# mit-han-lab/TinyChatEngine

Hardware: AMD Instinct MI355X
Metric: decode tokens/s (W4A16 linears of one token, M=1) + GEMV GB/s vs HBM roofline (higher is better)
Workload: dtype int4 weights x fp16 activations, fp32 accumulate; 1 GPU; W4A16 decode GEMV M=1, llama3-8b (true shapes, model.h:83): 32 blocks x [qkv [4096, 1024, 1024], o 4096, gate/up 14336, down] + lm_head 128256, group 128; parallelism=single GPU, issue=one hipGraph replay per token (129 launches in stream order)

## Files before the change

### tinychatengine_amd/csrc/tce_capi.hip

```cpp
#include <hip/hip_runtime.h>

#include <cstdarg>
#include <cstdio>
#include <cstring>
#include <new>
#include <algorithm>
#include <string>
#include <vector>

#include "tce_common.hpp"
#include "w4a16_kernels.hpp"

namespace tce {
int launch_w8a8(const tce_w8a8_desc &d, hipStream_t stream, hipError_t *hip_err, void *scratch = nullptr, char *describe = nullptr, int describe_len = 0);
size_t w8a8_scratch_bytes();
void set_w8a8_xsplit(int xs);
}

namespace {

thread_local char g_err[512] = "";
thread_local int g_gemv_rows = 0, g_gemv_wn = 0, g_gemv_wk = 0, g_gemv_depth = 0;
thread_local int g_gemm_mt = 0, g_gemm_nt = 0;
thread_local int g_debug_mode_capi = 0;
void *g_dbg_buf_capi = nullptr;

int fail(int code, const char *fmt, ...) __attribute__((format(printf, 2, 3)));
int fail(int code, const char *fmt, ...) {
    va_list ap;
    va_start(ap, fmt);
    vsnprintf(g_err, sizeof(g_err), fmt, ap);
    va_end(ap);
    return code;
}

int hip_fail(hipError_t e, const char *what) {
    return fail(TCE_ERR_HIP, "%s: %s", what, hipGetErrorString(e));
}

int check_w4a16(const tce_w4a16_desc *d) {
    if (!d) return fail(TCE_ERR_BAD_ARG, "null descriptor");
    if (!d->A || !d->qweight || !d->scales || !d->zeros || !d->C) return fail(TCE_ERR_BAD_ARG, "null data pointer");
    if (d->M <= 0 || d->N <= 0 || d->K <= 0) return fail(TCE_ERR_BAD_ARG, "non-positive M/N/K (%d,%d,%d)", d->M, d->N, d->K);
    if (d->group_size != 128 && d->group_size != 64 && d->group_size != 32)
        return fail(TCE_ERR_UNSUPPORTED_GROUP, "Unsupported group size: %d", d->group_size);
    if (d->K % d->group_size != 0 || d->K % 32 != 0)
        return fail(TCE_ERR_UNSUPPORTED_SHAPE, "K=%d must be a multiple of the group size and of 32", d->K);
    const int lda = d->lda ? d->lda : d->K;
    if (lda % 8 != 0 || reinterpret_cast<uintptr_t>(d->A) % 16 != 0)
        return fail(TCE_ERR_UNSUPPORTED_SHAPE, "A must be 16-byte aligned with lda %% 8 == 0");
    if (reinterpret_cast<uintptr_t>(d->qweight) % 16 != 0) return fail(TCE_ERR_UNSUPPORTED_SHAPE, "qweight must be 16-byte aligned");
    if (d->flags & TCE_W4_SILU_MUL_PAIRS) {
        if (d->N % 2 != 0) return fail(TCE_ERR_UNSUPPORTED_SHAPE, "TCE_W4_SILU_MUL_PAIRS needs an even N (interleaved gate/up rows), got %d", d->N);
        if (d->flags & (TCE_W4_ADD_TO_C | TCE_W4_FORCE_GEMM)) return fail(TCE_ERR_BAD_ARG, "TCE_W4_SILU_MUL_PAIRS cannot be combined with ADD_TO_C / FORCE_GEMM");
    }
    if (d->rmsnorm_gamma && (d->flags & TCE_W4_FORCE_GEMM)) return fail(TCE_ERR_BAD_ARG, "rmsnorm_gamma cannot be combined with TCE_W4_FORCE_GEMM");
    return TCE_OK;
}

}

extern "C" {

int tce_version(void) { return TCE_VERSION; }
const char *tce_last_error(void) { return g_err; }
const char *tce_build_info(void) { return "tce_hip gfx950 wave64 hipcc " __VERSION__; }

int64_t tce_w4a16_algorithmic_bytes(int M, int N, int K, int G) {
    const int64_t nk = (int64_t)N * K;
    return nk / 2 + 2 * nk / G + nk / (2 * (int64_t)G) + 2 * (int64_t)M * K + 2 * (int64_t)M * N;
}

thread_local int g_pk_mode = 0;
constexpr int kPkMinM = 129;

static bool use_pk(const tce_w4a16_desc *d, bool want_gemm) {
    if (!d->prepacked || g_pk_mode == 9 || !want_gemm || d->K % 128 != 0 || d->rmsnorm_gamma) return false;
    if (g_pk_mode >= 1 && g_pk_mode <= 8) return true;
    if (d->M < kPkMinM || g_gemm_mt != 0) return false;
    if (d->flags & TCE_W4_SILU_MUL_PAIRS) return true;
    if (d->group_size != 128) return true;
    const bool has_scratch = d->scratch != nullptr && (reinterpret_cast<uintptr_t>(d->scratch) & 255) == 0;
    return tce::gemm_pk_estimate_us(d->M, d->N, d->K, nullptr, has_scratch, nullptr, d->group_size, (d->flags & TCE_W4_ZERO_POINT_IS_8) != 0) < tce::gemm_dma_estimate_us(d->M, d->N, d->K) + 1.5f;
}

constexpr long long kPersistentMinWeights = 1LL << 62;
constexpr long long kFusedNormPersistentRows = 16384;
thread_local int g_gemv_kernel = 0;
thread_local int g_skinny_enabled = 1;

int tce_w4a16_set_gemv_config(int rows, int wn, int wk, int depth) {
    if (rows == 0 && wn == 0 && wk == 0) {
        g_gemv_rows = g_gemv_wn = g_gemv_wk = g_gemv_depth = 0;
        g_gemv_kernel = 0;
        tce::set_gemv_stream_config(0, 0, 0);
        return TCE_OK;
    }
    if (wk == 0) {
        if ((rows % 10 != 0 && rows % 10 != 1 && rows % 10 != 2 && rows % 10 != 4) || rows < 0 || rows >= 90 || wn < 1 || wn > 16 || (depth != 0 && depth != 2 && depth != 3))
            return fail(TCE_ERR_BAD_ARG, "stream GEMV config rows=%d waves=%d depth=%d is not available", rows, wn, depth);
        tce::set_gemv_stream_config(rows, wn, depth);
        g_gemv_kernel = 2;
        return TCE_OK;
    }
    const int dd = depth ? depth : 2;
    if (!tce::gemv_variant_exists(rows, wn, wk, dd))
        return fail(TCE_ERR_BAD_ARG, "GEMV variant rows=%d wn=%d wk=%d depth=%d was not compiled", rows, wn, wk, dd);
    g_gemv_rows = rows;
    g_gemv_wn = wn;
    g_gemv_wk = wk;
    g_gemv_depth = dd;
    g_gemv_kernel = 1;
    return TCE_OK;
}

int tce_w4a16_set_gemv_i8(int mode, int rows) {
    if (mode < 0 || mode > 1 || rows < 0 || rows > 2) return fail(TCE_ERR_BAD_ARG, "tce_w4a16_set_gemv_i8: mode %d rows %d", mode, rows);
    tce::set_gemv_i8_mode(mode, rows);
    return TCE_OK;
}

int tce_attention_set_tuning(int waves_per_workgroup, int workgroups, int heads_per_workgroup) {
    const bool ok = (waves_per_workgroup == 0 || waves_per_workgroup == 4 || waves_per_workgroup == 8 || waves_per_workgroup == 16) &&
                    (workgroups == 0 || (workgroups >= 32 && workgroups <= 8192)) &&
                    (heads_per_workgroup == 0 || heads_per_workgroup == 1 || heads_per_workgroup == 2 || heads_per_workgroup == 4);
    if (!ok) return fail(TCE_ERR_BAD_ARG, "tce_attention_set_tuning(%d, %d, %d)", waves_per_workgroup, workgroups, heads_per_workgroup);
    tce::set_attention_fast_waves(waves_per_workgroup);
    tce::set_attention_fast_target(workgroups);
    tce::set_attention_fast_fuse(heads_per_workgroup);
    return TCE_OK;
}

int tce_w8a8_set_tuning(int quartets_per_tile, int big_tiles, int deep_pipeline) {
    const bool ok = (quartets_per_tile == 0 || quartets_per_tile == 1 || quartets_per_tile == 2 || quartets_per_tile == 4) &&
                    ((big_tiles >= 0 && big_tiles <= 4) || big_tiles == 9) &&
                    (deep_pipeline == 0 || deep_pipeline == 1 || deep_pipeline == 2 || deep_pipeline == 4 || deep_pipeline == 9);
    if (!ok) return fail(TCE_ERR_BAD_ARG, "tce_w8a8_set_tuning(%d, %d, %d)", quartets_per_tile, big_tiles, deep_pipeline);
    tce::set_w8a8_ksplit(quartets_per_tile);
    tce::set_w8a8_big(big_tiles);
    tce::set_w8a8_deep(deep_pipeline);
    return TCE_OK;
}

static thread_local int g_plan_eager = 0;
int tce_w4a16_set_debug_mode(int mode) {
    if (mode >= 50000 && mode <= 50499) {
        tce::set_gemv_ovl_config((mode - 50000) % 100, (mode - 50000) / 100);
        return TCE_OK;
    }
    if (mode == 2930 || mode == 2931) {
        tce::set_attention_fast_probe_no_combine(mode - 2930);
        return TCE_OK;
    }
    if (mode >= 2920 && mode <= 2924) {
        tce::set_attention_fast_fuse(mode - 2920);
        return TCE_OK;
    }
    if (mode >= 2900 && mode <= 2916) {
        tce::set_attention_fast_waves(mode - 2900);
        return TCE_OK;
    }
    const bool pk_mode_in_attention_range = (mode >= 6950 && mode <= 6958) || (mode >= 6972 && mode <= 6974) || (mode >= 7700 && mode <= 7710 + 512) || mode == 6916 || mode == 6917;
    if (mode >= 3000 && mode <= 3000 + 8192 && !pk_mode_in_attention_range) {
        tce::set_attention_fast_target(mode - 3000);
        return TCE_OK;
    }
    if (mode >= 1000 && mode <= 1256) {
        tce::set_skinny_max_m(mode - 1000);
        return TCE_OK;
    }
    if (mode >= 2700 && mode <= 2899 && ((mode - 2700) % 100 == 0 || (mode - 2700) % 100 == 4 || (mode - 2700) % 100 == 8)) {
        tce::set_attention_prefill_waves((mode >= 2800 ? 200 : 100) + (mode % 100));
        return TCE_OK;
    }
    if (mode == 2950 || mode == 2954 || mode == 2958 || mode == 2964 || mode == 2968) {
        tce::set_attention_prefill_waves(mode - 2950);
        return TCE_OK;
    }
    if ((mode >= 75 && mode <= 78) || mode == 176 || mode == 177) {
        tce::set_w8a8_big(mode == 78 ? 9 : (mode >= 176 ? mode - 173 : mode - 75));
        return TCE_OK;
    }
    if (mode >= 7710 && mode <= 7710 + 512) {
        tce::set_i8_token_max_units(mode - 7710);
        return TCE_OK;
    }
    if (mode >= 7700 && mode <= 7703) {
        if (mode <= 7701) tce::set_i8_token_mode(mode - 7700);
        else {
#ifndef TCE_LAB
            if (mode == 7702) return fail(TCE_ERR_BAD_ARG, "debug mode 7702 (per-stage stamps of the token kernel) needs the lab build (python -m tinychatengine_amd.build --lab, TCE_LIB_PATH)");
#endif
            tce::set_i8_token_stamps(mode == 7702 ? g_dbg_buf_capi : nullptr);
        }
        return TCE_OK;
    }
    if (mode >= 19000 && mode <= 19999) {
        tce::set_w8a8_kslice(mode - 19000);
        return TCE_OK;
    }
    if (mode >= 190 && mode <= 192) {
        tce::set_w8a8_rows32(mode - 190);
        return TCE_OK;
    }
    if (mode >= 180 && mode <= 188) {
        tce::set_w8a8_xsplit(mode - 180);
        return TCE_OK;
    }
    if (mode == 170 || mode == 171 || mode == 172 || mode == 174 || mode == 179) {
        tce::set_w8a8_deep(mode - 170);
        return TCE_OK;
    }
    if (mode == 15000 || mode == 15001) {
        g_plan_eager = mode - 15000;
        return TCE_OK;
    }
    if (mode >= 70 && mode <= 74) {
        tce::set_w8a8_ksplit(mode - 70);
        return TCE_OK;
    }
    if (mode >= 640 && mode <= 644) {
        g_pk_mode = 4;
        tce::set_gemm_pk_ablation(0);
        tce::set_gemm_pk_mode(4, 0);
        tce::set_gemm_pk_split(mode - 640);
        return TCE_OK;
    }
#ifndef TCE_LAB
    if ((mode > 2600 && mode <= 2664) || (mode > 600 && mode <= 664) || (mode > 26000 && mode <= 26256) || mode == 1 || mode == 2 || mode == 4 || mode == 7702)
        return fail(TCE_ERR_BAD_ARG, "debug mode %d selects a diagnostic instantiation that only the lab build holds (python -m tinychatengine_amd.build --lab, TCE_LIB_PATH)", mode);
#endif
    if (mode >= 2600 && mode <= 2664) {
        g_pk_mode = mode == 2600 ? 0 : 6;
        tce::set_gemm_pk_mode(mode == 2600 ? 0 : 6, 0);
        tce::set_gemm_pk_ablation(mode - 2600);
        return TCE_OK;
    }
    if (mode >= 600 && mode <= 664) {
        g_pk_mode = mode == 600 ? 0 : 1;
        tce::set_gemm_pk_mode(mode == 600 ? 0 : 1, 0);
        tce::set_gemm_pk_ablation(mode - 600);
        return TCE_OK;
    }
    if (mode == 2676) {
        g_pk_mode = 8;
        tce::set_gemm_pk_ablation(0);
        tce::set_gemm_pk_split(0);
        tce::set_gemm_pk_mode(16, 0);
        return TCE_OK;
    }
    if (mode >= 51000 && mode <= 51016) {
        tce::set_gemv_i8_mixed_waves(mode - 51000);
        return TCE_OK;
    }
    if (mode == 6916 || mode == 6917) {
        tce::set_gemm_pk_form16_auto(mode - 6916);
        return TCE_OK;
    }
    if (mode == 2675) {
        g_pk_mode = 8;
        tce::set_gemm_pk_ablation(0);
        tce::set_gemm_pk_split(0);
        tce::set_gemm_pk_mode(15, 0);
        return TCE_OK;
    }
    if (mode == 2673 || mode == 2674) {
        g_pk_mode = 8;
        tce::set_gemm_pk_ablation(0);
        tce::set_gemm_pk_split(0);
        tce::set_gemm_pk_mode(mode - 2660, 0);
        return TCE_OK;
    }
    if (mode >= 2670 && mode <= 2672) {
        g_pk_mode = 8;
        tce::set_gemm_pk_ablation(0);
        tce::set_gemm_pk_split(0);
        tce::set_gemm_pk_mode(10 + mode - 2670, 0);
        return TCE_OK;
    }
    if (mode >= 2682 && mode <= 2684) {
        g_pk_mode = 8;
        tce::set_gemm_pk_ablation(0);
        tce::set_gemm_pk_mode(12, 0);
        tce::set_gemm_pk_split(mode - 2680);
        return TCE_OK;
    }
    if (mode >= 6950 && mode <= 6958) {
        tce::set_gemm_pk_handoff_delta(mode - 6950);
        return TCE_OK;
    }
    if (mode == 696 || mode == 697 || mode == 698 || (mode >= 6972 && mode <= 6974)) {
        tce::set_gemm_pk_prio(mode == 698 ? -1 : mode >= 6970 ? mode - 6970 : mode - 696);
        return TCE_OK;
    }
    if (mode == 694 || mode == 695) {
        tce::set_gemm_pk_handoff(mode - 694);
        return TCE_OK;
    }
    if (mode == 692 || mode == 693) {
        tce::set_gemm_pk_wide_auto(mode - 692);
        return TCE_OK;
    }
    if (mode >= 26000 && mode <= 26256) {
        g_pk_mode = mode == 26000 ? 0 : 8;
        tce::set_gemm_pk_mode(mode == 26000 ? 0 : 10, 0);
        tce::set_gemm_pk_ablation(mode - 26000);
        return TCE_OK;
    }
    if (mode == 2669) {
        g_pk_mode = 8;
        tce::set_gemm_pk_ablation(0);
        tce::set_gemm_pk_split(0);
        tce::set_gemm_pk_mode(9, 0);
        return TCE_OK;
    }
    if (mode >= 672 && mode <= 674) {
        g_pk_mode = 7;
        tce::set_gemm_pk_ablation(0);
        tce::set_gemm_pk_mode(7, 0);
        tce::set_gemm_pk_split(mode - 670);
        return TCE_OK;
    }
    if (mode == 690 || mode == 691) {
        tce::set_gemm_pk256_auto(mode - 690);
        return TCE_OK;
    }
    if (mode >= 60 && mode <= 69) {
        g_pk_mode = mode - 60;
        tce::set_gemm_pk_split(0);
        tce::set_gemm_pk_ablation(0);
        tce::set_gemm_pk_mode(g_pk_mode >= 1 && g_pk_mode <= 8 && g_pk_mode != 5 ? g_pk_mode : 0, 0);
        return TCE_OK;
    }
    if (mode >= 50 && mode <= 52) {
        tce::set_gemm_dma_mode(mode - 50);
        return TCE_OK;
    }
    if (mode == 40 || mode == 41 || mode == 42 || mode == 44 || mode == 48) {
        tce::set_gemm_xcd_rows(mode - 40);
        tce::set_gemm_dma_xcd_rows(mode - 40);
        return TCE_OK;
    }
    if (mode >= 45 && mode <= 47) {
        tce::set_gemv_shared_xsum(mode == 45 ? 2 : mode - 46);
        return TCE_OK;
    }
    if (mode >= 80 && mode <= 87) {
        tce::set_lnq_form(mode - 80);
        return TCE_OK;
    }
    if (mode >= 20 && mode <= 30) {
        g_skinny_enabled = mode != 29;
        tce::set_skinny_config(mode == 29 ? 0 : (mode == 30 ? 9 : mode - 20));
        return TCE_OK;
    }
    if (mode >= 10 && mode <= 12) {
        tce::set_gemv_order(mode - 10);
        return TCE_OK;
    }
    if (mode < 0 || mode > 4) return fail(TCE_ERR_BAD_ARG, "debug mode %d", mode);
    tce::set_gemv_debug_mode(mode);
    tce::set_gemv_stream_debug(mode, g_dbg_buf_capi);
    tce::set_gemv_ovl_stamps(mode == 2 ? g_dbg_buf_capi : nullptr);
    g_debug_mode_capi = mode;
    return TCE_OK;
}

int tce_w4a16_set_debug_buffer(void *buf) {
    tce::set_lnq_stamps(buf);
    tce::set_gemv_debug_buffer(buf);
    g_dbg_buf_capi = buf;
    tce::set_gemv_stream_debug(g_debug_mode_capi, buf);
    tce::set_gemv_ovl_stamps(g_debug_mode_capi == 2 ? buf : nullptr);
    return TCE_OK;
}

int tce_reset_last_error(void) {
    int first = 0;
    for (int i = 0; i < 8; ++i) {
        const hipError_t e = hipGetLastError();
        if (e == hipSuccess) break;
        if (!first) first = (int)e;
    }
    fail(TCE_OK, "");
    return first;
}

int tce_malloc(void **ptr, size_t bytes, int managed) {
    if (!ptr || bytes == 0) return fail(TCE_ERR_BAD_ARG, "tce_malloc: bad argument");
    const hipError_t e = managed ? hipMallocManaged(ptr, bytes, hipMemAttachGlobal) : hipMalloc(ptr, bytes);
    return e == hipSuccess ? TCE_OK : hip_fail(e, managed ? "hipMallocManaged" : "hipMalloc");
}

int tce_free(void *ptr) {
    if (!ptr) return TCE_OK;
    const hipError_t e = hipFree(ptr);
    return e == hipSuccess ? TCE_OK : hip_fail(e, "hipFree");
}

int tce_host_alloc(void **ptr, size_t bytes) {
    if (!ptr || bytes == 0) return fail(TCE_ERR_BAD_ARG, "tce_host_alloc: bad argument");
    const hipError_t e = hipHostMalloc(ptr, bytes, hipHostMallocMapped | hipHostMallocCoherent);
    return e == hipSuccess ? TCE_OK : hip_fail(e, "hipHostMalloc");
}

int tce_host_free(void *ptr) {
    if (!ptr) return TCE_OK;
    const hipError_t e = hipHostFree(ptr);
    return e == hipSuccess ? TCE_OK : hip_fail(e, "hipHostFree");
}

int tce_memcpy(void *dst, const void *src, size_t bytes, int kind, void *stream) {
    if (!dst || !src) return fail(TCE_ERR_BAD_ARG, "tce_memcpy: null pointer");
    const hipMemcpyKind k = kind == TCE_MEMCPY_H2D ? hipMemcpyHostToDevice : (kind == TCE_MEMCPY_D2H ? hipMemcpyDeviceToHost : hipMemcpyDeviceToDevice);
    const hipError_t e = hipMemcpyAsync(dst, src, bytes, k, static_cast<hipStream_t>(stream));
    return e == hipSuccess ? TCE_OK : hip_fail(e, "hipMemcpyAsync");
}

int tce_synchronize(void *stream) {
    const hipError_t e = stream ? hipStreamSynchronize(static_cast<hipStream_t>(stream)) : hipDeviceSynchronize();
    return e == hipSuccess ? TCE_OK : hip_fail(e, "synchronize");
}

int tce_device_count(void) {
    int n = 0;
    return hipGetDeviceCount(&n) == hipSuccess ? n : 0;
}

int tce_w4a16_gemv_variant(int idx, int *rows, int *wn, int *wk, int *depth) {
    static const int table[][4] = {
#define TCE_V(R, N_, K_, D_) {R, N_, K_, D_},
        TCE_GEMV_VARIANTS(TCE_V)
#undef TCE_V
    };
    const int n = (int)(sizeof(table) / sizeof(table[0]));
    if (idx < 0 || idx >= n || !rows || !wn || !wk || !depth) return TCE_ERR_BAD_ARG;
    *rows = table[idx][0];
    *wn = table[idx][1];
    *wk = table[idx][2];
    *depth = table[idx][3];
    return TCE_OK;
}

int tce_w4a16_gemm_variant(int idx, int *mt, int *nt) {
    static const int table[][2] = {
#define TCE_V(M_, N_) {M_, N_}, {100 + M_, N_}, {200 + M_, N_},
        TCE_GEMM_VARIANTS(TCE_V)
#undef TCE_V
    };
    const int n = (int)(sizeof(table) / sizeof(table[0]));
    if (idx < 0 || idx >= n || !mt || !nt) return TCE_ERR_BAD_ARG;
    *mt = table[idx][0];
    *nt = table[idx][1];
    return TCE_OK;
}

int tce_w4a16_set_gemm_config(int mt, int nt) {
    if (mt == 0 && nt == 0) {
        g_gemm_mt = g_gemm_nt = 0;
        return TCE_OK;
    }
    if (!tce::gemm_variant_exists(mt >= 200 ? mt - 200 : mt, nt)) return fail(TCE_ERR_BAD_ARG, "GEMM variant %dx%d was not compiled", mt, nt);
    g_gemm_mt = mt;
    g_gemm_nt = nt;
    return TCE_OK;
}

static int forward_group_norm(const tce_w4a16_desc *descs, int count, const float *gamma, float eps, void *stream) {
    if (!descs || count < 1 || count > TCE_MAX_GROUP) return fail(TCE_ERR_BAD_ARG, "group count %d not in 1..%d", count, TCE_MAX_GROUP);
    if (!gamma || reinterpret_cast<uintptr_t>(gamma) % 16 != 0) return fail(TCE_ERR_BAD_ARG, "gamma must be a 16-byte aligned fp32 [K] vector");
    for (int i = 0; i < count; ++i) {
        const int rc = check_w4a16(&descs[i]);
        if (rc != TCE_OK) return rc;
        const tce_w4a16_desc &a = descs[0], &b = descs[i];
        if (b.M != a.M || b.K != a.K || b.group_size != a.group_size || b.A != a.A || b.lda != a.lda)
            return fail(TCE_ERR_BAD_ARG, "grouped linears must share M, K, group size and the activation");
    }
    if (descs[0].M != 1) return fail(TCE_ERR_UNSUPPORTED_SHAPE, "the fused RMSNorm prologue is a decode (M = 1) path; use tce_rmsnorm_half for M = %d", descs[0].M);
    hipError_t he = hipSuccess;
    if (g_gemv_kernel == 0 && g_debug_mode_capi == 0 && tce::gemv_i8_supports(descs, count, true)) {
        const int rc = tce::launch_w4a16_gemv_i8(descs, count, static_cast<hipStream_t>(stream), &he, gamma, eps);
        if (rc == TCE_OK) return TCE_OK;
        if (rc == TCE_ERR_HIP) return hip_fail(he, "w4a16 gemv (int8 contraction, rmsnorm prologue) launch");
        if (rc != TCE_ERR_UNSUPPORTED_SHAPE) return fail(rc, "w4a16 gemv (int8 contraction, rmsnorm prologue): unsupported configuration");
    }
    long long rows = 0;
    for (int i = 0; i < count; ++i) rows += descs[i].N;
// ... 897 lines not shown
    return rc == TCE_OK ? TCE_OK : fail(rc, "%s: unsupported shape", who);
}

int tce_layernorm_q_w8a8_group(const float *x, const float *ln_weight, const float *ln_bias, int m, int k, const tce_w8a8_desc *lin, int count,
                               void *ln_out, void *stream) {
    if (!x || !ln_weight || !ln_bias || !lin) return fail(TCE_ERR_BAD_ARG, "tce_layernorm_q_w8a8_group: null pointer");
    if (m < 1 || m > 8) return fail(TCE_ERR_UNSUPPORTED_SHAPE, "tce_layernorm_q_w8a8_group is a decode path: 1 <= m <= 8, got %d", m);
    if (k <= 0 || k % 16 != 0) return fail(TCE_ERR_UNSUPPORTED_SHAPE, "tce_layernorm_q_w8a8_group: k=%d must be a positive multiple of 16", k);
    if (count < 1 || count > TCE_MAX_GROUP) return fail(TCE_ERR_BAD_ARG, "group count %d not in 1..%d", count, TCE_MAX_GROUP);
    if ((reinterpret_cast<uintptr_t>(x) & 15)) return fail(TCE_ERR_UNSUPPORTED_SHAPE, "x must be 16-byte aligned");
    for (int i = 0; i < count; ++i) {
        const tce_w8a8_desc &d = lin[i];
        if (!d.B || !d.C || d.N <= 0) return fail(TCE_ERR_BAD_ARG, "linear %d: null B / C or non-positive N", i);
        if (d.M != m || d.K != k || d.batch != 1 || d.b_per_row) return fail(TCE_ERR_BAD_ARG, "linear %d: M / K must be the normalised rows', batch 1, no per-row B", i);
        if ((reinterpret_cast<uintptr_t>(d.B) & 15)) return fail(TCE_ERR_UNSUPPORTED_SHAPE, "linear %d: B must be 16-byte aligned", i);
        const bool ok = (d.out_kind == TCE_OUT_INT8 && (d.bias_kind == TCE_BIAS_INT8 || d.bias_kind == TCE_BIAS_NONE)) ||
                        (d.out_kind == TCE_OUT_FP32 && (d.bias_kind == TCE_BIAS_FP32 || d.bias_kind == TCE_BIAS_NONE));
        if (!ok) return fail(TCE_ERR_UNSUPPORTED_KIND, "linear %d: bias_kind %d with out_kind %d has no reference counterpart", i, d.bias_kind, d.out_kind);
        if (d.bias_kind != TCE_BIAS_NONE && !d.bias) return fail(TCE_ERR_BAD_ARG, "linear %d: bias_kind set but bias is null", i);
        if (d.out_kind == TCE_OUT_INT8 && (d.q_min < -128 || d.q_max > 127 || d.q_min > d.q_max)) return fail(TCE_ERR_BAD_ARG, "linear %d: q_min/q_max out of int8 range", i);
    }
    hipError_t he = hipSuccess;
    const int rc = tce::launch_lnq_w8a8_group(x, ln_weight, ln_bias, m, k, lin, count, ln_out, static_cast<hipStream_t>(stream), &he);
    if (rc == TCE_ERR_HIP) return hip_fail(he, "layernorm_q + w8a8 launch");
    if (rc != TCE_OK) return fail(rc, "tce_layernorm_q_w8a8_group: the rows do not fit the CU's LDS (m * k too large)");
    return TCE_OK;
}

struct TunedGeometry {
    int rows = 0, wn = 0, wk = 0, depth = 0;
    int shared_xsum = 0;
    int order = 0;
};

struct tce_plan {
    std::vector<tce_w4a16_desc> descs;
    std::vector<int32_t> groups;
    hipGraph_t graph = nullptr;
    hipGraphExec_t exec = nullptr;
    tce::TokenPlan *token = nullptr;
    tce::I8TokenPlan *token_i8 = nullptr;
    int token_i8_taken = 0;
    std::vector<TunedGeometry> tuned;
};

static void plan_free(tce_plan *p) {
    if (!p) return;
    if (p->exec) (void)hipGraphExecDestroy(p->exec);
    if (p->graph) (void)hipGraphDestroy(p->graph);
    tce::token_plan_destroy(p->token);
    tce::i8_token_plan_destroy(p->token_i8);
    delete p;
}


static std::string launch_signature(const tce_w4a16_desc *d, int count) {
    char buf[64];
    std::string s;
    std::snprintf(buf, sizeof buf, "M%d K%d G%d n%d", d[0].M, d[0].K, d[0].group_size, count);
    s = buf;
    for (int j = 0; j < count; ++j) {
        std::snprintf(buf, sizeof buf, " N%d f%x", d[j].N, (unsigned)d[j].flags);
        s += buf;
    }
    s += d[0].rmsnorm_gamma ? " norm" : "";
    return s;
}

static int tune_plan_launches(const std::vector<tce_w4a16_desc> &descs, const std::vector<int32_t> &groups, std::vector<TunedGeometry> &out) {
    const int n_launches = (int)groups.size();
    out.assign(n_launches, TunedGeometry{});
    std::vector<std::string> sig(n_launches);
    std::vector<int> offs(n_launches);
    std::vector<tce_w4a16_desc> copy(descs);
    size_t scratch_halves = 0;
    for (int i = 0, off = 0; i < n_launches; off += groups[i], ++i) {
        offs[i] = off;
        const tce_w4a16_desc *d = &descs[off];
        if (d->M == 1 && !(d->flags & TCE_W4_FORCE_GEMM) && !tce::gemv_i8_supports(d, groups[i], d->rmsnorm_gamma != nullptr)) sig[i] = launch_signature(d, groups[i]);
        size_t need = 0;
        for (int j = 0; j < groups[i]; ++j) need += (((size_t)(d[j].ldc ? d[j].ldc : d[j].N) * d[j].M + 127) & ~(size_t)127) + 128;
        scratch_halves = need > scratch_halves ? need : scratch_halves;
    }
    void *scratch = nullptr;
    hipStream_t st = nullptr;
    hipEvent_t e0 = nullptr, e1 = nullptr;
    if (hipMalloc(&scratch, scratch_halves * 2 + 256) != hipSuccess) return TCE_OK;
    if (hipStreamCreateWithFlags(&st, hipStreamNonBlocking) != hipSuccess || hipEventCreate(&e0) != hipSuccess || hipEventCreate(&e1) != hipSuccess) {
        (void)hipFree(scratch);
        if (st) (void)hipStreamDestroy(st);
        if (e0) (void)hipEventDestroy(e0);
        return TCE_OK;
    }
    (void)hipMemsetAsync(scratch, 0, scratch_halves * 2 + 256, st);
    for (int i = 0; i < n_launches; ++i) {
        size_t at = 0;
        for (int j = 0; j < groups[i]; ++j) {
            tce_w4a16_desc &d = copy[offs[i] + j];
            d.C = static_cast<char *>(scratch) + at * 2;
            at += (((size_t)(d.ldc ? d.ldc : d.N) * d.M + 127) & ~(size_t)127) + 128;
        }
    }
    auto time_plan = [&](const std::vector<TunedGeometry> &g) -> float {
        hipGraph_t graph = nullptr;
        hipGraphExec_t exec = nullptr;
        if (hipStreamBeginCapture(st, hipStreamCaptureModeThreadLocal) != hipSuccess) return -1.f;
        int rc = TCE_OK;
        for (int i = 0; i < n_launches && rc == TCE_OK; ++i) {
            const bool forced = g[i].rows != 0;
            if (forced && tce_w4a16_set_gemv_config(g[i].rows, g[i].wn, g[i].wk, g[i].depth) != TCE_OK) rc = TCE_ERR_BAD_ARG;
            tce::set_gemv_shared_xsum(g[i].shared_xsum);
            tce::set_gemv_order(g[i].order);
            if (rc == TCE_OK) rc = groups[i] == 1 ? tce_w4a16_forward(&copy[offs[i]], st) : tce_w4a16_forward_group(&copy[offs[i]], groups[i], st);
            tce::set_gemv_order(0);
            tce::set_gemv_shared_xsum(0);
            if (forced) (void)tce_w4a16_set_gemv_config(0, 0, 0, 0);
        }
        const hipError_t ee = hipStreamEndCapture(st, &graph);
        float us = -1.f;
        if (rc == TCE_OK && ee == hipSuccess && hipGraphInstantiate(&exec, graph, nullptr, nullptr, 0) == hipSuccess) {
            bool ok = true;
            for (int w = 0; w < 3 && ok; ++w) ok = hipGraphLaunch(exec, st) == hipSuccess;
            ok = ok && hipStreamSynchronize(st) == hipSuccess;
            for (int round = 0; ok && round < 3; ++round) {
                (void)hipEventRecord(e0, st);
                for (int r = 0; r < 10 && ok; ++r) ok = hipGraphLaunch(exec, st) == hipSuccess;
                (void)hipEventRecord(e1, st);
                ok = ok && hipEventSynchronize(e1) == hipSuccess;
                float ms = 0.f;
                if (ok && hipEventElapsedTime(&ms, e0, e1) == hipSuccess) us = us < 0.f ? ms * 100.f : std::min(us, ms * 100.f);
            }
            if (!ok) us = -1.f;
        }
        if (exec) (void)hipGraphExecDestroy(exec);
        if (graph) (void)hipGraphDestroy(graph);
        (void)hipGetLastError();
        return us;
    };
    static const int cands[][4] = {{2, 4, 1, 2}, {3, 4, 1, 2}, {4, 4, 1, 1}, {2, 8, 1, 2}, {2, 4, 1, 1}, {2, 4, 1, 3}, {4, 4, 1, 2}, {1, 4, 1, 2}, {1, 4, 1, 1}, {4, 8, 1, 1},
                                   {2, 16, 0, 0}, {22, 8, 0, 3}, {4, 16, 0, 0}};
    const int ncand = (int)(sizeof cands / sizeof cands[0]);
    std::vector<TunedGeometry> best(n_launches);
    float best_us = time_plan(best);
    std::vector<char> done(n_launches, 0);
    for (int i = 0; i < n_launches && best_us > 0.f; ++i) {
        if (sig[i].empty() || done[i]) continue;
        std::vector<int> members;
        for (int k = i; k < n_launches; ++k)
            if (sig[k] == sig[i]) {
                members.push_back(k);
                done[k] = 1;
            }
        for (int c = 0; c < ncand; ++c) {
            if (cands[c][2] != 0 && !tce::gemv_variant_exists(cands[c][0], cands[c][1], cands[c][2], cands[c][3])) continue;
            std::vector<TunedGeometry> trial(best);
            for (int k : members) trial[k] = TunedGeometry{cands[c][0], cands[c][1], cands[c][2], cands[c][3]};
            const float us = time_plan(trial);
            if (us > 0.f && us < 0.993f * best_us) {
                best_us = us;
                best = trial;
            }
        }
    }
    for (int knob = 0; knob < 3; ++knob) {
        std::fill(done.begin(), done.end(), 0);
        for (int i = 0; i < n_launches && best_us > 0.f; ++i) {
            if (sig[i].empty() || done[i]) continue;
            std::vector<TunedGeometry> trial(best);
            for (int k = i; k < n_launches; ++k)
                if (sig[k] == sig[i]) {
                    if (knob == 0) trial[k].shared_xsum = 2;
                    else trial[k].order = knob;
                    done[k] = 1;
                }
            const float us = time_plan(trial);
            if (us > 0.f && us < 0.993f * best_us) {
                best_us = us;
                best = trial;
            }
        }
    }
    out = best;
    (void)tce_w4a16_set_gemv_config(0, 0, 0, 0);
    (void)hipStreamSynchronize(st);
    (void)hipEventDestroy(e0);
    (void)hipEventDestroy(e1);
    (void)hipStreamDestroy(st);
    (void)hipFree(scratch);
    tce_reset_last_error();
    return TCE_OK;
}

int tce_plan_create_ex(const tce_w4a16_desc *descs, const int32_t *group_sizes, int n_launches, int flags, tce_plan **out) {
    if (!descs || !group_sizes || n_launches < 1 || !out) return fail(TCE_ERR_BAD_ARG, "bad argument");
    if (flags & ~(TCE_PLAN_CHAINED | TCE_PLAN_TAGGED | TCE_PLAN_OVERLAPPED | TCE_PLAN_TUNED | TCE_PLAN_INDEPENDENT)) return fail(TCE_ERR_BAD_ARG, "unknown plan flags 0x%x", flags);
    const bool independent = (flags & TCE_PLAN_INDEPENDENT) != 0;
    if (independent && flags != TCE_PLAN_INDEPENDENT) return fail(TCE_ERR_BAD_ARG, "TCE_PLAN_INDEPENDENT does not combine with other plan flags (0x%x)", flags);
    const int max_group = independent ? TCE_MAX_INDEPENDENT : TCE_MAX_GROUP;
    tce_plan *p = new (std::nothrow) tce_plan();
    if (!p) return fail(TCE_ERR_BAD_ARG, "out of host memory");
    int total = 0;
    for (int i = 0; i < n_launches; ++i) {
        if (group_sizes[i] < 1 || group_sizes[i] > max_group) {
            delete p;
            return fail(TCE_ERR_BAD_ARG, "group size %d not in 1..%d", group_sizes[i], max_group);
        }
        total += group_sizes[i];
    }
    p->descs.assign(descs, descs + total);
    p->groups.assign(group_sizes, group_sizes + n_launches);

    bool chained = (flags & (TCE_PLAN_CHAINED | TCE_PLAN_TAGGED | TCE_PLAN_OVERLAPPED)) && n_launches > 1 && (g_gemv_kernel != 1 || (flags & TCE_PLAN_OVERLAPPED));
    for (int i = 0, off = 0; i < n_launches && chained; off += p->groups[i], ++i)
        for (int j = 0; j < p->groups[i] && chained; ++j) {
            const tce_w4a16_desc &a = p->descs[off], &b = p->descs[off + j];
            if (check_w4a16(&b) != TCE_OK || b.M != a.M || b.K != a.K || b.group_size != a.group_size || b.A != a.A || b.lda != a.lda ||
                b.rmsnorm_gamma != a.rmsnorm_gamma || (a.rmsnorm_gamma && b.rmsnorm_eps != a.rmsnorm_eps) ||
                (b.flags & TCE_W4_FORCE_GEMM))
                chained = false;
        }
    hipError_t he = hipSuccess;
    if (chained && (flags & TCE_PLAN_TAGGED) && !(flags & TCE_PLAN_OVERLAPPED)) {
        const int rc = tce::i8_token_plan_create(p->descs.data(), p->groups.data(), n_launches, &p->token_i8, &p->token_i8_taken, &he);
        if (rc == TCE_ERR_HIP) {
            plan_free(p);
            return hip_fail(he, "int8 token plan");
        }
        if (rc != TCE_OK) p->token_i8 = nullptr;
        else chained = false;
    }
    if (chained) {
        const int rc = tce::token_plan_create(p->descs.data(), p->groups.data(), n_launches, &p->token, &he, (flags & TCE_PLAN_OVERLAPPED) ? 1 : 0);
        if (rc == TCE_ERR_HIP) {
            plan_free(p);
            return hip_fail(he, "token plan");
        }
        if (rc != TCE_OK) p->token = nullptr;
    }

    if ((flags & TCE_PLAN_TUNED) && !p->token && !p->token_i8 && g_gemv_kernel == 0) (void)tune_plan_launches(p->descs, p->groups, p->tuned);
    hipStream_t cap = nullptr;
    hipError_t e = hipStreamCreateWithFlags(&cap, hipStreamNonBlocking);
    if (e != hipSuccess) {
        plan_free(p);
        return hip_fail(e, "hipStreamCreate");
    }
    e = hipStreamBeginCapture(cap, hipStreamCaptureModeThreadLocal);
    if (e != hipSuccess) {
        (void)hipStreamDestroy(cap);
        plan_free(p);
        return hip_fail(e, "hipStreamBeginCapture");
    }
    int rc = TCE_OK;
    if (p->token) {
        rc = tce::token_plan_enqueue(p->token, cap, &he);
    } else {
        if (p->token_i8) rc = tce::i8_token_plan_enqueue(p->token_i8, cap, &he);
        for (int i = 0, off = 0; i < n_launches && rc == TCE_OK; off += p->groups[i], ++i) {
            if (i < p->token_i8_taken) continue;
            const bool forced = i < (int)p->tuned.size() && p->tuned[i].rows != 0;
            if (forced) (void)tce_w4a16_set_gemv_config(p->tuned[i].rows, p->tuned[i].wn, p->tuned[i].wk, p->tuned[i].depth);
            if (i < (int)p->tuned.size()) {
                tce::set_gemv_shared_xsum(p->tuned[i].shared_xsum);
                tce::set_gemv_order(p->tuned[i].order);
            }
            if (independent) rc = tce_w4a16_forward_independent(&p->descs[off], p->groups[i], nullptr, cap);
            else rc = p->groups[i] == 1 ? tce_w4a16_forward(&p->descs[off], cap) : tce_w4a16_forward_group(&p->descs[off], p->groups[i], cap);
            tce::set_gemv_order(0);
            tce::set_gemv_shared_xsum(0);
            if (forced) (void)tce_w4a16_set_gemv_config(0, 0, 0, 0);
        }
    }
    e = hipStreamEndCapture(cap, &p->graph);
    (void)hipStreamDestroy(cap);
    if (rc != TCE_OK) {
        plan_free(p);
        return rc == TCE_ERR_HIP && he != hipSuccess ? hip_fail(he, "token kernel launch") : rc;
    }
    if (e != hipSuccess) {
        plan_free(p);
        return hip_fail(e, "hipStreamEndCapture");
    }
    e = hipGraphInstantiate(&p->exec, p->graph, nullptr, nullptr, 0);
    if (e != hipSuccess) {
        plan_free(p);
        return hip_fail(e, "hipGraphInstantiate");
    }
    *out = p;
    return TCE_OK;
}

int tce_plan_create(const tce_w4a16_desc *descs, const int32_t *group_sizes, int n_launches, tce_plan **out) {
    return tce_plan_create_ex(descs, group_sizes, n_launches, 0, out);
}

int tce_plan_is_chained(const tce_plan *plan) {
    if (plan && plan->token_i8) return 4;
    return plan && plan->token ? (tce::token_plan_mode(plan->token) == 1 ? 3 : 2) : 0;
}

int tce_plan_geometry(const tce_plan *plan, int *rows, int *depth, int *waves, int *workgroups) {
    if (plan && plan->token_i8 && rows && depth && waves && workgroups) {
        *rows = plan->token_i8_taken;
        *depth = 1;
        *waves = 16;
        *workgroups = tce::i8_token_plan_blocks(plan->token_i8);
        return TCE_OK;
    }
    if (!plan || !plan->token || !rows || !depth || !waves || !workgroups) return fail(TCE_ERR_BAD_ARG, "not a chained plan");
    tce::token_plan_geometry(plan->token, rows, depth, waves, workgroups);
    return TCE_OK;
}

int tce_plan_launch_geometry(const tce_plan *plan, int launch, int *rows, int *waves_n, int *waves_k, int *depth) {
    if (!plan || launch < 0 || launch >= (int)plan->groups.size() || !rows || !waves_n || !waves_k || !depth) return fail(TCE_ERR_BAD_ARG, "tce_plan_launch_geometry: bad argument");
    const TunedGeometry g = launch < (int)plan->tuned.size() ? plan->tuned[launch] : TunedGeometry{};
    *rows = g.rows;
    *waves_n = g.wn;
    *waves_k = g.wk;
    *depth = g.depth + 100 * g.shared_xsum + 1000 * g.order;
    return TCE_OK;
}

int tce_plan_status(tce_plan *plan) {
    if (!plan) return fail(TCE_ERR_BAD_ARG, "null plan");
    hipError_t e = hipDeviceSynchronize();
    if (e != hipSuccess) return hip_fail(e, "hipDeviceSynchronize");
    if (plan->token_i8) {
        unsigned st8 = 0;
        if (tce::i8_token_plan_status(plan->token_i8, &st8, &e) != TCE_OK) return hip_fail(e, "hipMemcpy");
        return st8 == 0 ? TCE_OK : fail(TCE_ERR_HIP, "tagged plan: a wait for activations timed out");
    }
    if (!plan->token) return TCE_OK;
    unsigned status = 0;
    if (tce::token_plan_status(plan->token, &status, &e) != TCE_OK) return hip_fail(e, "hipMemcpy");
    return status == 0 ? TCE_OK : fail(TCE_ERR_HIP, "chained plan: a device-wide barrier timed out");
}

int tce_plan_launch(tce_plan *plan, void *stream) {
    if (!plan || !plan->exec) return fail(TCE_ERR_BAD_ARG, "null plan");
    if (g_plan_eager && !plan->token && !plan->token_i8) {
        int rc = TCE_OK;
        const int n_launches = (int)plan->groups.size();
        for (int i = 0, off = 0; i < n_launches && rc == TCE_OK; off += plan->groups[i], ++i)
            rc = plan->groups[i] == 1 ? tce_w4a16_forward(&plan->descs[off], stream) : tce_w4a16_forward_group(&plan->descs[off], plan->groups[i], stream);
        return rc;
    }
    const hipError_t e = hipGraphLaunch(plan->exec, static_cast<hipStream_t>(stream));
    return e == hipSuccess ? TCE_OK : hip_fail(e, "hipGraphLaunch");
}

int tce_plan_n_launches(const tce_plan *plan) { return plan ? (int)plan->groups.size() : 0; }

void tce_plan_destroy(tce_plan *plan) { plan_free(plan); }

}
```

### tinychatengine_amd/csrc/w4a16_gemv_i8_token.hip

```cpp
#include "tce_common.hpp"
#include "w4a16_kernels.hpp"
#include "w4a16_mfma_layout.hpp"

#include <new>
#include <vector>

namespace tce {

namespace {

constexpr int kTokWaves = 16;
constexpr int kTokMaxChunks = 15;
constexpr int kTokMaxUnits = 512;
constexpr int kTokMaxTiles = 128;

struct TokSeg {
    const void *words;
    const half_t *dscales;
    half_t *C;
    unsigned *C_tag;
    int N, epilogue, tile_begin, bytes_w, bytes_s, pad;
};
static_assert(sizeof(TokSeg) == 56, "record layout");
struct TokStage {
    const half_t *A;
    const unsigned *A_tag;
    int K, U, nch, nseg, ntiles, pad;
    TokSeg seg[TCE_MAX_GROUP];
};
constexpr int kRecWords = sizeof(TokStage) / 4;
static_assert(sizeof(TokStage) % 8 == 0 && kRecWords <= 128, "a record is fetched by one wave, 8 bytes per lane");

struct TokArgs {
    const TokStage *stages;
    int n_stages;
    unsigned *status;
    const unsigned *epoch;
    unsigned long long *dbg;
};

constexpr int kPlanesBytes = kTokMaxChunks * 4096;
constexpr int kRecOff = kPlanesBytes;
constexpr int kShOff = kRecOff + 3 * (int)sizeof(TokStage);
constexpr int kCntOff = kShOff + 128;
constexpr int kRedOff = kCntOff + kTokMaxTiles * 4;
constexpr int kLdsBytes = kRedOff + kTokMaxUnits * 64;

template <int DPP_CTRL, int ROW_MASK = 0xF>
__device__ __forceinline__ unsigned tok_dpp_max_u32(unsigned v) {
    const unsigned t = (unsigned)__builtin_amdgcn_update_dpp(0, (int)v, DPP_CTRL, ROW_MASK, 0xF, false);
    return v > t ? v : t;
}
template <int DPP_CTRL>
__device__ __forceinline__ float tok_dpp_add_f32(float v) {
    const int t = __builtin_amdgcn_update_dpp(0, __builtin_bit_cast(int, v), DPP_CTRL, 0xF, 0xF, false);
    return v + __builtin_bit_cast(float, t);
}
template <int DPP_CTRL>
__device__ __forceinline__ unsigned tok_dpp_u32(unsigned v) {
    return (unsigned)__builtin_amdgcn_update_dpp(0, (int)v, DPP_CTRL, 0xF, 0xF, false);
}
__device__ __forceinline__ int sgpr(int v) { return __builtin_amdgcn_readfirstlane(v); }
template <typename T>
__device__ __forceinline__ T *sgpr_ptr(T *p) {
    const unsigned long long u = reinterpret_cast<unsigned long long>(p);
    const unsigned lo = (unsigned)__builtin_amdgcn_readfirstlane((int)(unsigned)u), hi = (unsigned)__builtin_amdgcn_readfirstlane((int)(unsigned)(u >> 32));
    return reinterpret_cast<T *>(((unsigned long long)hi << 32) | lo);
}

template <bool STAMPS>
__global__ __launch_bounds__(64 * kTokWaves) void w4a16_gemv_i8_token_kernel(const TokArgs args) {
    extern __shared__ __attribute__((aligned(16))) unsigned char smem[];
    const int tid = threadIdx.x;
    const int lane = tid & 63;
    const int w = __builtin_amdgcn_readfirstlane(tid >> 6);
    const int kq = lane >> 4, j16 = lane & 15;
    const int p_l = j16 & 3, uu_l = j16 >> 2;
    const int P = gridDim.x, b = blockIdx.x;
    const int n = args.n_stages;
    unsigned *const planes_all = reinterpret_cast<unsigned *>(smem);
    TokStage *const rec = reinterpret_cast<TokStage *>(smem + kRecOff);
    int *const shx = reinterpret_cast<int *>(smem + kShOff);
    unsigned *const tile_cnt = reinterpret_cast<unsigned *>(smem + kCntOff);
    float *const red = reinterpret_cast<float *>(smem + kRedOff);
    const unsigned tag = (unsigned)__builtin_amdgcn_readfirstlane((int)__hip_atomic_load(args.epoch, __ATOMIC_RELAXED, __HIP_MEMORY_SCOPE_AGENT)) << 16;
    unsigned long long *const stamps = STAMPS && args.dbg ? args.dbg + (size_t)b * n * 8 : nullptr;
    auto stamp = [&](int s, int i) {
        if constexpr (STAMPS) {
            if (stamps && tid == 0) stamps[s * 8 + i] = wall_clock64();
        }
    };

    if (tid < kRecWords) reinterpret_cast<unsigned *>(&rec[0])[tid] = reinterpret_cast<const unsigned *>(args.stages)[tid];
    __syncthreads();

    uint4_t wq[8];
    uint2_t sc[2];
    const int4_t zero4 = int4_t{0, 0, 0, 0};

    for (int s = 0; s < n; ++s) {
        const TokStage *R = &rec[s % 3];
        const int K = sgpr(R->K), U = sgpr(R->U), nch = sgpr(R->nch), nseg = sgpr(R->nseg), ntiles = sgpr(R->ntiles);
        const int ntw = b < ntiles ? (ntiles - 1 - b) / P + 1 : 0;
        const int nunits = ntw * nch;
        stamp(s, 0);

        const int rec_pair = (lane * 2 < kRecWords ? lane * 2 : kRecWords - 2);
        const uint2_t recv = *reinterpret_cast<const uint2_t *>(reinterpret_cast<const unsigned *>(args.stages + (s + 1 < n ? s + 1 : n - 1)) + rec_pair);

        auto seg_of = [&](int t) {
            int si = 0;
            for (int q = 1; q < nseg; ++q)
                if (t >= sgpr(R->seg[q].tile_begin)) si = q;
            return si;
        };
        auto request = [&](int u) {
            const int i = u / nch, c = u - i * nch;
            const int t = b + i * P;
            const TokSeg *S = &R->seg[seg_of(t)];
            const int tl = t - sgpr(S->tile_begin);
            const int u0 = c * 8;
            const __amdgpu_buffer_rsrc_t rs_w = __builtin_amdgcn_make_buffer_rsrc(const_cast<void *>(sgpr_ptr(S->words)), 0, sgpr(S->bytes_w), 0x00020000);
            const __amdgpu_buffer_rsrc_t rs_none = __builtin_amdgcn_make_buffer_rsrc(const_cast<void *>(sgpr_ptr(S->words)), 0, 0, 0x00020000);
            const __amdgpu_buffer_rsrc_t rs_s = __builtin_amdgcn_make_buffer_rsrc(const_cast<half_t *>(sgpr_ptr(S->dscales)), 0, sgpr(S->bytes_s), 0x00020000);
#pragma unroll
            for (int ps = 0; ps < 2; ++ps) {
                const int ga = tl * U + u0 + ps * 4 + uu_l;
                sc[ps] = __builtin_bit_cast(uint2_t, __builtin_amdgcn_raw_buffer_load_b64(rs_s, (ga * 16 + 4 * kq) * 2, 0, 0));
            }
#pragma unroll
            for (int tt = 0; tt < 8; ++tt)
                wq[tt] = __builtin_amdgcn_raw_buffer_load_b128(u0 + tt < U ? rs_w : rs_none, lane * 16, (tl * U + u0 + tt) * 1024,  2);
        };
        int u_cur = w;
        const int u_first = u_cur;
        if (u_cur < nunits) request(u_cur);
        __builtin_amdgcn_sched_barrier(0);

        uint4_t xv[2];
        xv[0] = xv[1] = uint4_t{0u, 0u, 0u, 0u};
        if (w < nch) {
            const unsigned *A_tag = sgpr_ptr(R->A_tag);
            if (A_tag == nullptr) {
                const __amdgpu_buffer_rsrc_t rs_x = __builtin_amdgcn_make_buffer_rsrc(const_cast<half_t *>(sgpr_ptr(R->A)), 0, K * 2, 0x00020000);
#pragma unroll
                for (int c = 0; c < 2; ++c) xv[c] = __builtin_amdgcn_raw_buffer_load_b128(rs_x, w * 2048 + (lane + 64 * c) * 16, 0, 0);
            } else {
                const __amdgpu_buffer_rsrc_t rs_t = __builtin_amdgcn_make_buffer_rsrc(const_cast<unsigned *>(A_tag), 0, K * 4, 0x00020000);
                bool need[2];
                uint4_t lo[2], hi[2];
#pragma unroll
                for (int c = 0; c < 2; ++c) {
                    need[c] = w * 1024 + (lane + 64 * c) * 8 < K;
                    lo[c] = hi[c] = uint4_t{tag, tag, tag, tag};
                }
                int tries = 0;
                for (;;) {
#pragma unroll
                    for (int c = 0; c < 2; ++c)
                        if (need[c]) {
                            lo[c] = __builtin_amdgcn_raw_buffer_load_b128(rs_t, w * 4096 + (lane + 64 * c) * 32, 0,  17);
                            hi[c] = __builtin_amdgcn_raw_buffer_load_b128(rs_t, w * 4096 + (lane + 64 * c) * 32 + 16, 0,  17);
                        }
                    bool again = false;
#pragma unroll
                    for (int c = 0; c < 2; ++c)
                        if (need[c]) {
                            const unsigned bad = ((lo[c].x ^ tag) | (lo[c].y ^ tag) | (lo[c].z ^ tag) | (lo[c].w ^ tag) | (hi[c].x ^ tag) | (hi[c].y ^ tag) | (hi[c].z ^ tag) |
                                                  (hi[c].w ^ tag)) >> 16;
                            need[c] = bad != 0u;
                            again |= need[c];
                        }
                    if (!__builtin_amdgcn_ballot_w64(again)) break;
                    __builtin_amdgcn_s_sleep(2);
                    if ((++tries & 255) == 0) {
                        if (__hip_atomic_load(args.status, __ATOMIC_RELAXED, __HIP_MEMORY_SCOPE_AGENT) != 0u) break;
                        if (tries > (1 << 18)) {
                            __hip_atomic_store(args.status, 1u, __ATOMIC_RELAXED, __HIP_MEMORY_SCOPE_AGENT);
                            break;
                        }
                    }
                }
#pragma unroll
                for (int c = 0; c < 2; ++c)
                    xv[c] = uint4_t{(lo[c].x & 0xFFFFu) | (lo[c].y << 16), (lo[c].z & 0xFFFFu) | (lo[c].w << 16), (hi[c].x & 0xFFFFu) | (hi[c].y << 16),
                                    (hi[c].z & 0xFFFFu) | (hi[c].w << 16)};
            }
            asm volatile("" : "+v"(xv[0]), "+v"(xv[1]));
        }
        stamp(s, 1);
        lds_barrier();
        stamp(s, 2);
        if (tid < kTokMaxTiles) tile_cnt[tid] = 0u;
        if (w < nch) {
            unsigned mx = 0;
#pragma unroll
            for (int c = 0; c < 2; ++c)
#pragma unroll
                for (int q = 0; q < 4; ++q) {
                    const unsigned v = xv[c][q] & 0x7FFF7FFFu;
                    const unsigned v2 = v << 16;
                    const unsigned m2 = v > v2 ? v : v2;
                    mx = mx > m2 ? mx : m2;
                }
            mx = tok_dpp_max_u32<0x111>(mx);
            mx = tok_dpp_max_u32<0x112>(mx);
            mx = tok_dpp_max_u32<0x114>(mx);
            mx = tok_dpp_max_u32<0x118>(mx);
            mx = tok_dpp_max_u32<0x142, 0xA>(mx);
            mx = tok_dpp_max_u32<0x143, 0xC>(mx);
            const int E = (int)((unsigned)__builtin_amdgcn_readlane((int)mx, 63) >> 26);
            const int sh = 44 - E;
            if (lane == 0) {
                shx[w] = sh;
                shx[16 + w] = E == 31 ? 1 : 0;
            }
            const float scale = __builtin_bit_cast(float, (unsigned)(127 + sh) << 23);
            unsigned *planes = planes_all + w * 1024;
#pragma unroll
            for (int c = 0; c < 2; ++c) {
                unsigned d[8];
#pragma unroll
                for (int q = 0; q < 4; ++q) {
                    const half_t lo = __builtin_bit_cast(half_t, (unsigned short)(xv[c][q] & 0xFFFFu));
                    const half_t hi = __builtin_bit_cast(half_t, (unsigned short)(xv[c][q] >> 16));
                    d[2 * q] = ((unsigned)(int)__builtin_fmaf((float)lo, scale, 0.0f) + 0x00808080u) ^ 0x00808080u;
                    d[2 * q + 1] = ((unsigned)(int)__builtin_fmaf((float)hi, scale, 0.0f) + 0x00808080u) ^ 0x00808080u;
                }
                const int cc = lane + 64 * c;
                const int tu = cc >> 4, sw = (cc >> 2) & 3, q4 = cc & 3;
#pragma unroll
                for (int h = 0; h < 2; ++h) {
                    const unsigned a0 = d[2 * h], a1 = d[2 * h + 4], a2 = d[2 * h + 1], a3 = d[2 * h + 5];
                    const unsigned t0 = __builtin_amdgcn_perm(a1, a0, 0x05010400u);
                    const unsigned t1 = __builtin_amdgcn_perm(a1, a0, 0x07030602u);
                    const unsigned t2 = __builtin_amdgcn_perm(a3, a2, 0x05010400u);
                    const unsigned t3 = __builtin_amdgcn_perm(a3, a2, 0x07030602u);
                    const int base = (((tu * 2 + h) * 4) * 4 + q4) * 4 + sw;
                    planes[base + 0] = __builtin_amdgcn_perm(t2, t0, 0x05040100u);
                    planes[base + 16] = __builtin_amdgcn_perm(t2, t0, 0x07060302u);
                    planes[base + 32] = __builtin_amdgcn_perm(t3, t1, 0x05040100u);
                    planes[base + 48] = __builtin_amdgcn_perm(t3, t1, 0x07060302u);
                }
            }
        }
        lds_barrier();
        stamp(s, 3);
        *reinterpret_cast<uint2_t *>(reinterpret_cast<unsigned *>(&rec[(s + 1) % 3]) + rec_pair) = recv;

        while (u_cur < nunits) {
            const int i = u_cur / nch, c = u_cur - i * nch;
            const unsigned *planes = planes_all + c * 1024;
            int4_t B[4][2];
#pragma unroll
            for (int uu = 0; uu < 4; ++uu) B[uu][0] = B[uu][1] = zero4;
            auto read_b = [&](int ps) {
#pragma unroll
                for (int uu = 0; uu < 4; ++uu)
                    if (uu_l == uu) {
#pragma unroll
                        for (int h = 0; h < 2; ++h) {
                            const unsigned *src = planes + (((((ps * 4 + uu) * 2 + h) * 4 + p_l) * 4 + kq) * 4);
                            B[uu][h] = __builtin_bit_cast(int4_t, *reinterpret_cast<const uint4_t *>(src));
                        }
                    }
            };
            read_b(0);
            if constexpr (STAMPS) {
                if (u_cur == u_first) {
                    asm volatile("s_waitcnt vmcnt(0)" ::: "memory");
                    stamp(s, 5);
                }
            }
            float acc[4] = {0.f, 0.f, 0.f, 0.f};
#pragma unroll
            for (int ps = 0; ps < 2; ++ps) {
                int4_t dd0 = zero4, dd1 = zero4;
#pragma unroll
                for (int uu = 0; uu < 4; ++uu) {
                    const int t = ps * 4 + uu;
                    int4_t alo, ahi;
#pragma unroll
                    for (int q = 0; q < 4; ++q) {
                        const unsigned x = wq[t][q];
                        ahi[q] = (int)((x & 0xF0F0F0F0u) ^ 0x80808080u);
                        alo[q] = (int)(((x << 4) & 0xF0F0F0F0u) ^ 0x80808080u);
                    }
                    dd0 = __builtin_amdgcn_mfma_i32_16x16x64_i8(alo, B[uu][0], dd0, 0, 0, 0);
                    dd1 = __builtin_amdgcn_mfma_i32_16x16x64_i8(ahi, B[uu][1], dd1, 0, 0, 0);
                }
                const half_t s0 = __builtin_bit_cast(half_t, (unsigned short)(sc[ps][0] & 0xFFFFu));
                const half_t s1 = __builtin_bit_cast(half_t, (unsigned short)(sc[ps][0] >> 16));
                const half_t s2 = __builtin_bit_cast(half_t, (unsigned short)(sc[ps][1] & 0xFFFFu));
                const half_t s3 = __builtin_bit_cast(half_t, (unsigned short)(sc[ps][1] >> 16));
                const int4_t tot = dd0 + dd1;
                acc[0] = __builtin_fmaf((float)tot[0], (float)s0, acc[0]);
                acc[1] = __builtin_fmaf((float)tot[1], (float)s1, acc[1]);
                acc[2] = __builtin_fmaf((float)tot[2], (float)s2, acc[2]);
                acc[3] = __builtin_fmaf((float)tot[3], (float)s3, acc[3]);
                if (ps == 0) read_b(1);
            }
            const int sh_c = sgpr(shx[c]);
            const bool bad_c = sgpr(shx[16 + c]) != 0;
            const float cj = bad_c ? __builtin_nanf("") : __builtin_bit_cast(float, (unsigned)(127 + 8 * p_l - sh_c - 4) << 23);
            float *slot = red + (size_t)u_cur * 16;
            if constexpr (STAMPS) {
                if (u_cur == u_first) {
                    asm volatile("" : "+v"(acc[0]), "+v"(acc[1]), "+v"(acc[2]), "+v"(acc[3]));
                    stamp(s, 6);
                }
            }
#pragma unroll
            for (int q = 0; q < 4; ++q) {
                float v = acc[q] * cj;
                v = tok_dpp_add_f32<0xB1>(v);
                v = tok_dpp_add_f32<0x4E>(v);
                v = tok_dpp_add_f32<0x128>(v);
                v = tok_dpp_add_f32<0x124>(v);
                if (j16 == 0) slot[kq * 4 + q] = v;
            }
            asm volatile("s_waitcnt lgkmcnt(0)" ::: "memory");
            unsigned old = 0;
            if (lane == 0) old = __hip_atomic_fetch_add(tile_cnt + i, 1u, __ATOMIC_RELAXED, __HIP_MEMORY_SCOPE_WORKGROUP);
            asm volatile("" ::: "memory");
            const bool last = (unsigned)__builtin_amdgcn_readfirstlane((int)old) == (unsigned)(nch - 1);
            if constexpr (STAMPS) {
                if (u_cur == u_first) stamp(s, 7);
            }
            const int t = b + i * P;
            if (last) {
                if constexpr (STAMPS) {
                    if (stamps && lane == 0) stamps[s * 8 + 4] = wall_clock64();
                }
                const TokSeg *S = &R->seg[seg_of(t)];
                const int tl = t - sgpr(S->tile_begin);
                const int N = sgpr(S->N), epi = sgpr(S->epilogue);
                half_t *C = sgpr_ptr(S->C);
                unsigned *C_tag = sgpr_ptr(S->C_tag);
                const float *parts = red + (size_t)(i * nch) * 16 + (lane & 15);
                float v = 0.f;
                for (int k2 = 0; k2 < nch; ++k2) v += parts[k2 * 16];
                const int row = tl * 16 + (lane & 15);
                half_t y = (half_t)v;
                const half_t y_other = __builtin_bit_cast(half_t, (unsigned short)tok_dpp_u32<0xB1>((unsigned)__builtin_bit_cast(unsigned short, y)));
                int idx = row;
                bool live = lane < 16 && row < N;
                if (epi & TCE_W4_SILU_MUL_PAIRS) {
                    y = silu_mul_half(y, y_other);
                    idx = row >> 1;
                    live = live && (lane & 1) == 0;
                } else if (epi & TCE_W4_ADD_TO_C) {
                    unsigned short oldc = 0;
                    if (live) oldc = __hip_atomic_load(reinterpret_cast<unsigned short *>(C) + row, __ATOMIC_RELAXED, __HIP_MEMORY_SCOPE_AGENT);
                    y = __builtin_bit_cast(half_t, oldc) + y;
                }
                const unsigned short bits = __builtin_bit_cast(unsigned short, y);
                if (live) {
                    if (epi & TCE_W4_ADD_TO_C) __hip_atomic_store(reinterpret_cast<unsigned short *>(C) + idx, bits, __ATOMIC_RELAXED, __HIP_MEMORY_SCOPE_AGENT);
                    else C[idx] = y;
                }
                if (C_tag) {
                    const unsigned word = tag | bits;
                    const __amdgpu_buffer_rsrc_t rs_c = __builtin_amdgcn_make_buffer_rsrc(C_tag, 0, 0x7FFFFFF0, 0x00020000);
                    if (epi & TCE_W4_SILU_MUL_PAIRS) {
                        const unsigned w1 = tok_dpp_u32<0x102>(word), w2 = tok_dpp_u32<0x104>(word), w3 = tok_dpp_u32<0x106>(word);
                        if (lane < 16 && (lane & 7) == 0 && row + 7 < N) {
                            __builtin_amdgcn_raw_buffer_store_b128(uint4_t{word, w1, w2, w3}, rs_c, idx * 4, 0,  17);
                        } else if (lane < 16 && row < N && (lane & 1) == 0 && !(((row & ~7) + 7) < N)) {
                            __hip_atomic_store(C_tag + idx, word, __ATOMIC_RELAXED, __HIP_MEMORY_SCOPE_AGENT);
                        }
                    } else {
                        const unsigned w1 = tok_dpp_u32<0x101>(word), w2 = tok_dpp_u32<0x102>(word), w3 = tok_dpp_u32<0x103>(word);
                        if (lane < 16 && (lane & 3) == 0 && row + 3 < N) {
                            __builtin_amdgcn_raw_buffer_store_b128(uint4_t{word, w1, w2, w3}, rs_c, idx * 4, 0,  17);
                        } else if (lane < 16 && row < N && !(((row & ~3) + 3) < N)) {
                            __hip_atomic_store(C_tag + idx, word, __ATOMIC_RELAXED, __HIP_MEMORY_SCOPE_AGENT);
                        }
                    }
                }
            }
            u_cur += kTokWaves;
            if (u_cur < nunits) request(u_cur);
        }
    }
}

__global__ void i8_token_epoch_kernel(unsigned *epoch) { *epoch = *epoch % 65535u + 1u; }

int tok_num_cus() {
    int dev = 0, cus = 0;
    if (hipGetDevice(&dev) != hipSuccess) return 0;
    if (hipDeviceGetAttribute(&cus, hipDeviceAttributeMultiprocessorCount, dev) != hipSuccess) return 0;
    return cus;
}

thread_local unsigned long long *g_tok_stamps = nullptr;
thread_local int g_tok_mode = 0;
thread_local int g_tok_max_units = kTokMaxUnits;

}

struct I8TokenPlan {
    TokStage *stages = nullptr;
    unsigned *sync = nullptr;
    unsigned *shadow = nullptr;
    int n = 0, blocks = 0;
    unsigned long long *stamps = nullptr;
};

void set_i8_token_stamps(void *buf) { g_tok_stamps = static_cast<unsigned long long *>(buf); }
void set_i8_token_mode(int mode) { g_tok_mode = mode == 1 ? 1 : 0; }
void set_i8_token_max_units(int u) { g_tok_max_units = u >= 1 && u <= kTokMaxUnits ? u : kTokMaxUnits; }

void i8_token_plan_destroy(I8TokenPlan *tp) {
    if (!tp) return;
    if (tp->stages) (void)hipFree(tp->stages);
    if (tp->sync) (void)hipFree(tp->sync);
    if (tp->shadow) (void)hipFree(tp->shadow);
    delete tp;
}

int i8_token_plan_stages(const I8TokenPlan *tp) { return tp ? tp->n : 0; }
int i8_token_plan_blocks(const I8TokenPlan *tp) { return tp ? tp->blocks : 0; }

int i8_token_plan_create(const tce_w4a16_desc *descs, const int32_t *groups, int n_launches, I8TokenPlan **out, int *n_taken, hipError_t *hip_err) {
    if (g_tok_mode == 1) return TCE_ERR_UNSUPPORTED_SHAPE;
    const int cus = tok_num_cus();
    if (cus == 0) return TCE_ERR_HIP;
#ifdef TCE_LAB
    const void *kfn = g_tok_stamps ? reinterpret_cast<const void *>(w4a16_gemv_i8_token_kernel<true>) : reinterpret_cast<const void *>(w4a16_gemv_i8_token_kernel<false>);
#else
    const void *kfn = reinterpret_cast<const void *>(w4a16_gemv_i8_token_kernel<false>);
#endif
    hipError_t e = hipFuncSetAttribute(kfn, hipFuncAttributeMaxDynamicSharedMemorySize, kLdsBytes);
    int per_cu = 0;
    if (e == hipSuccess) e = hipOccupancyMaxActiveBlocksPerMultiprocessor(&per_cu, kfn, 64 * kTokWaves, kLdsBytes);
    if (e != hipSuccess) {
        if (hip_err) *hip_err = e;
        return TCE_ERR_HIP;
    }
    if (per_cu < 1) return TCE_ERR_UNSUPPORTED_SHAPE;
    const int P = cus;

    std::vector<TokStage> host;
    std::vector<int> first_desc;
    for (int l = 0, off = 0; l < n_launches; off += groups[l], ++l) {
        const tce_w4a16_desc &d0 = descs[off];
        bool ok = d0.M == 1 && d0.group_size == 128 && d0.K % 128 == 0 && d0.K >= 128 && (d0.K + 1023) / 1024 <= kTokMaxChunks && !d0.rmsnorm_gamma &&
                  (d0.lda == 0 || d0.lda == d0.K) && groups[l] <= TCE_MAX_GROUP;
        TokStage st{};
        int tiles = 0;
        for (int i = 0; i < groups[l] && ok; ++i) {
            const tce_w4a16_desc &d = descs[off + i];
            ok = d.M == 1 && d.K == d0.K && d.group_size == 128 && d.A == d0.A && d.prepacked && !(reinterpret_cast<uintptr_t>(d.prepacked) & 255) && (d.flags & TCE_W4_ZERO_POINT_IS_8) &&
                 !(d.flags & TCE_W4_FORCE_GEMM) && !d.rmsnorm_gamma && (long long)pk::nt16(d.N) * (d.K / 2) * 16 < (1LL << 31) && !(d.flags & ~(TCE_W4_ZERO_POINT_IS_8 | TCE_W4_SILU_MUL_PAIRS | TCE_W4_ADD_TO_C));
            if ((d.flags & TCE_W4_SILU_MUL_PAIRS) && (d.N % 2 != 0 || (d.flags & TCE_W4_ADD_TO_C))) ok = false;
            if (!ok) break;
            TokSeg &sg = st.seg[i];
            const unsigned char *base = static_cast<const unsigned char *>(d.prepacked);
            sg.words = base;
            sg.dscales = reinterpret_cast<const half_t *>(base + pk::dscales_offset(d.N, d.K, d.group_size));
            sg.C = static_cast<half_t *>(d.C);
            sg.C_tag = nullptr;
            sg.N = d.N;
            sg.epilogue = d.flags & (TCE_W4_SILU_MUL_PAIRS | TCE_W4_ADD_TO_C);
            sg.tile_begin = tiles;
            sg.bytes_w = (int)pk::words_bytes(d.N, d.K);
            sg.bytes_s = (int)pk::dscales_bytes(d.N, d.K, d.group_size);
            tiles += pk::nt16(d.N);
        }
        if (ok) {
            st.A = static_cast<const half_t *>(d0.A);
            st.A_tag = nullptr;
            st.K = d0.K;
            st.U = d0.K / 128;
            st.nch = (st.U + 7) / 8;
            st.nseg = groups[l];
            st.ntiles = tiles;
            for (int i = groups[l]; i < TCE_MAX_GROUP; ++i) st.seg[i] = st.seg[0];
            const int tiles_wg = (tiles + P - 1) / P;
            ok = tiles_wg <= kTokMaxTiles && tiles_wg * st.nch <= g_tok_max_units;
        }
        if (!ok) break;
        host.push_back(st);
        first_desc.push_back(off);
    }
    const int n = (int)host.size();
    if (n < 2) return TCE_ERR_UNSUPPORTED_SHAPE;

    I8TokenPlan *tp = new (std::nothrow) I8TokenPlan();
    if (!tp) return TCE_ERR_BAD_ARG;
    tp->n = n;
    tp->blocks = P;
#ifdef TCE_LAB
    tp->stamps = g_tok_stamps;
#endif
    auto n_out_of = [&](const TokStage &L, int i) { return (L.seg[i].epilogue & TCE_W4_SILU_MUL_PAIRS) ? L.seg[i].N / 2 : L.seg[i].N; };
    size_t words = 0;
    std::vector<size_t> base((size_t)n * TCE_MAX_GROUP, 0);
    for (int l = 0; l < n; ++l)
        for (int i = 0; i < host[l].nseg; ++i) {
            base[(size_t)l * TCE_MAX_GROUP + i] = words;
            words += ((size_t)n_out_of(host[l], i) + 63) & ~(size_t)63;
        }
    e = hipMalloc(reinterpret_cast<void **>(&tp->shadow), words * sizeof(unsigned));
    if (e == hipSuccess) e = hipMemset(tp->shadow, 0, words * sizeof(unsigned));
    std::vector<int> producer(n, -1);
    std::vector<std::vector<char>> consumed((size_t)n, std::vector<char>(TCE_MAX_GROUP, 0));
    bool refuse = false;
    for (int l = 0; l < n && e == hipSuccess && !refuse; ++l) {
        TokStage &L = host[l];
        const char *a0 = reinterpret_cast<const char *>(L.A), *a1 = a0 + (size_t)L.K * 2;
        for (int q = l - 1; q >= 0 && producer[l] < 0 && !refuse; --q)
            for (int i = 0; i < host[q].nseg; ++i) {
                const char *c0 = reinterpret_cast<const char *>(host[q].seg[i].C), *c1 = c0 + (size_t)n_out_of(host[q], i) * 2;
                if (a0 >= c0 && a1 <= c1) {
                    if ((a0 - c0) % 16 != 0) {
                        refuse = true;
                        break;
                    }
                    L.A_tag = tp->shadow + base[(size_t)q * TCE_MAX_GROUP + i] + (a0 - c0) / 2;
                    producer[l] = q;
                    consumed[q][i] = 1;
                    break;
                }
                if (a0 < c1 && a1 > c0) {
                    refuse = true;
                    break;
                }
            }
    }
    for (int l = 0; l < n; ++l)
        for (int i = 0; i < host[l].nseg; ++i) host[l].seg[i].C_tag = tp->shadow + base[(size_t)l * TCE_MAX_GROUP + i];
    if (e == hipSuccess && !refuse) {
        const size_t nw64 = ((size_t)n + 63) / 64;
        std::vector<uint64_t> anc((size_t)n * nw64, 0);
        for (int l = 0; l < n; ++l)
            if (producer[l] >= 0) {
                const int q = producer[l];
                for (size_t k = 0; k < nw64; ++k) anc[l * nw64 + k] = anc[q * nw64 + k];
                anc[l * nw64 + (size_t)q / 64] |= 1ull << (q % 64);
            }
        for (int l = 1; l < n && !refuse; ++l)
            for (int i = 0; i < host[l].nseg && !refuse; ++i) {
                const char *w0 = reinterpret_cast<const char *>(host[l].seg[i].C), *w1 = w0 + (size_t)n_out_of(host[l], i) * 2;
                for (int q = 0; q < l; ++q) {
                    bool touches = false;
                    if (producer[q] < 0) {
                        const char *r0 = reinterpret_cast<const char *>(host[q].A), *r1 = r0 + (size_t)host[q].K * 2;
                        touches = r0 < w1 && r1 > w0;
                    }
                    for (int k = 0; k < host[q].nseg && !touches; ++k) {
                        const char *c0 = reinterpret_cast<const char *>(host[q].seg[k].C), *c1 = c0 + (size_t)n_out_of(host[q], k) * 2;
                        touches = c0 < w1 && c1 > w0;
                    }
                    if (touches && !((anc[l * nw64 + (size_t)q / 64] >> (q % 64)) & 1ull)) {
                        refuse = true;
                        break;
                    }
                }
            }
    }
    if (refuse) {
        i8_token_plan_destroy(tp);
        return TCE_ERR_UNSUPPORTED_SHAPE;
    }
    if (e == hipSuccess) e = hipMalloc(reinterpret_cast<void **>(&tp->stages), sizeof(TokStage) * n);
    if (e == hipSuccess) e = hipMemcpy(tp->stages, host.data(), sizeof(TokStage) * n, hipMemcpyHostToDevice);
    if (e == hipSuccess) e = hipMalloc(reinterpret_cast<void **>(&tp->sync), sizeof(unsigned) * 2);
    if (e == hipSuccess) {
        const unsigned init[2] = {0u, 1u};
        e = hipMemcpy(tp->sync, init, sizeof(init), hipMemcpyHostToDevice);
    }
    if (e != hipSuccess) {
        if (hip_err) *hip_err = e;
        i8_token_plan_destroy(tp);
        return TCE_ERR_HIP;
    }
    *out = tp;
    *n_taken = n;
    return TCE_OK;
}

int i8_token_plan_enqueue(I8TokenPlan *tp, hipStream_t stream, hipError_t *hip_err) {
    TokArgs a;
    a.stages = tp->stages;
    a.n_stages = tp->n;
    a.status = tp->sync;
    a.epoch = tp->sync + 1;
    a.dbg = tp->stamps;
    const dim3 grid(tp->blocks), block(64 * kTokWaves);
#ifdef TCE_LAB
    if (tp->stamps) hipLaunchKernelGGL(w4a16_gemv_i8_token_kernel<true>, grid, block, kLdsBytes, stream, a);
    else
#endif
    hipLaunchKernelGGL(w4a16_gemv_i8_token_kernel<false>, grid, block, kLdsBytes, stream, a);
    hipLaunchKernelGGL(i8_token_epoch_kernel, dim3(1), dim3(1), 0, stream, tp->sync + 1);
    const hipError_t e = hipGetLastError();
    if (e != hipSuccess) {
        if (hip_err) *hip_err = e;
        return TCE_ERR_HIP;
    }
    return TCE_OK;
}

int i8_token_plan_status(I8TokenPlan *tp, unsigned *status, hipError_t *hip_err) {
    const hipError_t e = hipMemcpy(status, tp->sync, sizeof(unsigned), hipMemcpyDeviceToHost);
    if (e != hipSuccess) {
        if (hip_err) *hip_err = e;
        return TCE_ERR_HIP;
    }
    return TCE_OK;
}

}
```

### tinychatengine_amd/csrc/w4a16_kernels.hpp

```cpp
#pragma once
#include "tce_common.hpp"

namespace tce {

struct GemvSeg {
    const uint4_t *qweight;
    const half_t *scales;
    const unsigned *zeros;
    half_t *C;
    int N, ldc, scales_stride, zeros_stride;
    int bytes_w, bytes_s, bytes_z;
    int block_begin;
    int epilogue;
};

struct GemvArgs {
    const half_t *A;
    int lda, M, K, log2g;
    int nseg;
    unsigned long long *dbg;
    int zeros_are_8;
    const float *gamma;
    float eps;
    int shared_xsum;
    GemvSeg seg[TCE_MAX_GROUP];
};

#define TCE_GEMV_VARIANTS(X) \
    X(1, 4, 1, 1)            \
    X(2, 4, 1, 1)            \
    X(4, 4, 1, 1)            \
    X(1, 4, 1, 2)            \
    X(2, 4, 1, 2)            \
    X(4, 4, 1, 2)            \
    X(2, 4, 1, 3)            \
    X(3, 4, 1, 1)            \
    X(3, 4, 1, 2)            \
    X(2, 8, 1, 2)            \
    X(4, 8, 1, 1)            \
    X(1, 2, 2, 1)            \
    X(2, 2, 2, 1)            \
    X(2, 2, 2, 2)            \
    X(1, 2, 4, 1)

bool gemv_variant_exists(int rows, int wn, int wk, int depth);
void set_gemv_debug_mode(int mode);
void set_gemv_order(int force);
void set_w8a8_deep(int d);
void set_w8a8_rows32(int r);
void set_w8a8_kslice(int code);
void set_w8a8_big(int b);
void set_lnq_stamps(void *p);
void set_lnq_form(int f);
void set_gemv_shared_xsum(int on);
void set_gemv_debug_buffer(void *p);

struct StreamLaunch {
    const half_t *A;
    int K, log2g;
    int nseg;
    int n_rg;
    GemvSeg seg[TCE_MAX_GROUP];
    const float *gamma;
    float eps;
    const unsigned *A_tag;
    unsigned *C_tag[TCE_MAX_GROUP];
};
void set_gemv_stream_config(int rows, int nw, int depth);
void set_gemv_stream_debug(int mode, void *buf);
bool gemv_stream_supports(const tce_w4a16_desc *descs, int count);
int launch_w4a16_gemv_stream(const tce_w4a16_desc *descs, int count, hipStream_t stream, hipError_t *hip_err,
                             const float *gamma = nullptr, float eps = 0.f);
struct TokenPlan;
int token_plan_create(const tce_w4a16_desc *descs, const int32_t *groups, int n_launches, TokenPlan **out, hipError_t *hip_err, int mode = 0);
int token_plan_mode(const TokenPlan *tp);
struct OvlGeom {
    int wn, xb, depth, rows_per_block, grid, per_cu;
    bool z8;
    size_t lds;
};
int ovl_chains();
int ovl_geometry(const tce_w4a16_desc *descs, int count, int cus, int chains, OvlGeom *g, hipError_t *hip_err);
hipError_t ovl_enqueue(const StreamLaunch *L, const OvlGeom &g, const unsigned *epoch, unsigned *status, int launch_index, hipStream_t stream);
void set_gemv_ovl_config(int depth, int chains);
void set_gemv_ovl_stamps(void *buf);
int token_plan_enqueue(TokenPlan *tp, hipStream_t stream, hipError_t *hip_err);
int token_plan_status(TokenPlan *tp, unsigned *status, hipError_t *hip_err);
void token_plan_geometry(const TokenPlan *tp, int *rows, int *depth, int *waves, int *blocks);
void token_plan_destroy(TokenPlan *tp);
int launch_w4a16_gemv(const tce_w4a16_desc *descs, int count, int forced_rows, int forced_wn, int forced_wk,
                      int forced_depth, hipStream_t stream, hipError_t *hip_err, const float *gamma = nullptr, float eps = 0.f);

bool gemv_i8_supports(const tce_w4a16_desc *descs, int count, bool with_norm = false);
int gemv_i8_rows_per_pass(int M, int K, int group_size);
void set_gemv_i8_mode(int mode, int rows);
struct I8ResidualNorm {
    const float *gamma;
    float eps;
    void *xn_out;
    void *workspace;
};
struct AttnDeferred;
int launch_w4a16_gemv_i8(const tce_w4a16_desc *descs, int count, hipStream_t stream, hipError_t *hip_err, const float *gamma = nullptr, float eps = 0.f, const I8ResidualNorm *rn = nullptr,
                         const AttnDeferred *comb = nullptr, const int *comb_pos_dev = nullptr, int comb_pos = 0);

struct PeerGatherEpi;
bool gemv_i8_mixed_supports(const tce_w4a16_desc *descs, int count);
void gemv_i8_mixed_geometry(const tce_w4a16_desc *descs, int count, int *waves, int *workgroups);
void set_gemv_i8_mixed_waves(int w);
int launch_w4a16_gemv_i8_mixed(const tce_w4a16_desc *descs, int count, hipStream_t stream, hipError_t *hip_err, const PeerGatherEpi *gather = nullptr, int gathered = -1);
struct I8TokenPlan;
int i8_token_plan_create(const tce_w4a16_desc *descs, const int32_t *groups, int n_launches, I8TokenPlan **out, int *n_taken, hipError_t *hip_err);
int i8_token_plan_enqueue(I8TokenPlan *tp, hipStream_t stream, hipError_t *hip_err);
int i8_token_plan_status(I8TokenPlan *tp, unsigned *status, hipError_t *hip_err);
int i8_token_plan_stages(const I8TokenPlan *tp);
int i8_token_plan_blocks(const I8TokenPlan *tp);
void i8_token_plan_destroy(I8TokenPlan *tp);
void set_i8_token_stamps(void *buf);
void set_i8_token_max_units(int u);
void set_i8_token_mode(int mode);

#define TCE_GEMM_VARIANTS(X) \
    X(8, 1)                  \
    X(8, 2)                  \
    X(4, 2)                  \
    X(4, 1)                  \
    X(2, 2)                  \
    X(4, 4)                  \
    X(2, 4)
bool gemm_variant_exists(int m_tiles, int n_tiles);
void set_gemm_xcd_rows(int xm);
void set_gemm_dma_xcd_rows(int xm);
float gemm_dma_estimate_us(int M, int N, int K);
void gemm_dma_describe(int M, int N, bool g128, int *mt, int *nt, int *ks);
void set_gemm_dma_mode(int mode);
void set_w8a8_ksplit(int ks);
int launch_w4a16_gemm_dma(const tce_w4a16_desc &d, int m_tiles, int n_tiles, hipStream_t stream, hipError_t *hip_err);
int launch_w4a16_gemm(const tce_w4a16_desc &d, int forced_mt, int forced_nt, hipStream_t stream, hipError_t *hip_err);

size_t prepack_bytes(int N, int K, int G);
int launch_w4a16_prepack(const tce_w4a16_desc &d, void *out, hipStream_t stream, hipError_t *hip_err);
int launch_w4a16_gemm_pk(const tce_w4a16_desc &d, const void *packed, hipStream_t stream, hipError_t *hip_err);
void set_gemm_pk256_auto(int on);
void set_gemm_pk_wide_auto(int on);
void set_gemm_pk_form16_auto(int on);
void set_gemm_pk_handoff_delta(int d);
void set_gemm_pk_prio(int on);
void set_gemm_pk_handoff(int on);
float gemm_pk_estimate_us(int M, int N, int K, int *form_out, bool has_scratch = false, int *split_out = nullptr, int group_size = 128, bool zero_point_8 = false);
size_t gemm_pk_scratch_bytes();
void set_gemm_pk_split(int s);
void set_gemm_pk_mode(int ks, int xm);
void set_gemm_pk_ablation(int abl);

int check_zero_point_8(const void *zeros, long long n_words, hipError_t *hip_err);
int check_zero_point_8_async(const void *zeros, long long n_words, int *verdict, hipStream_t stream, hipError_t *hip_err);

int launch_awq_fp16acc(int M, int N, int K, int G, const void *A, const void *qweight, const void *scales, void *C,
                       hipStream_t stream, hipError_t *hip_err);
int launch_awq_repack(int N, int K, int G, const void *qweight, const void *scales, void *workspace, hipStream_t stream,
                      hipError_t *hip_err);

bool skinny_supports(const tce_w4a16_desc &d);
void set_skinny_config(int ks);
void set_skinny_max_m(int m);
int launch_w4a16_skinny(const tce_w4a16_desc &d, hipStream_t stream, hipError_t *hip_err);

int launch_layernorm_q(const float *x, const float *w, const float *b, void *out, int m, int n, hipStream_t stream, hipError_t *hip_err);
int launch_lnq_w8a8_group(const float *x, const float *ln_w, const float *ln_b, int m, int k, const tce_w8a8_desc *lin, int count, void *ln_out,
                          hipStream_t stream, hipError_t *hip_err);
int launch_opt_softmax_q(const float *scores, const float *mask, void *probs, int heads, int sq, int tgz, int ldp, hipStream_t stream, hipError_t *hip_err);
int launch_opt_kv_append(const void *k, const void *v, void *kc, void *vt, int heads, int hd, int sq, int pos, int max_keys, hipStream_t stream, hipError_t *hip_err);
int launch_rmsnorm_half(const void *x, const float *gamma, void *out, int m, int n, float eps, hipStream_t stream, hipError_t *hip_err);
int launch_bmm_f16t(const void *A, const void *B, void *C, int batch, int M, int N, int K, unsigned short alpha_bits, hipStream_t stream, hipError_t *hip_err);
int launch_attention_decode(const void *q, const void *K, const void *Vt, const void *mask, void *out, int heads, int t, int hd, unsigned short alpha_bits,
                            hipStream_t stream, hipError_t *hip_err);
struct Comm;
int comm_create(int rank, int world, int max_vector_elems, int slots, Comm **out, hipError_t *he);
int comm_export(Comm *c, void *handle64, hipError_t *he);
int comm_connect_ipc(Comm *c, const void *handles, hipError_t *he);
int comm_connect_local(Comm *c, Comm *const *all, hipError_t *he);
int comm_set_timeout_ms(Comm *c, int ms);
int comm_reset(Comm *c, hipError_t *he);
int comm_device(const Comm *c);
int comm_status(Comm *c, hipError_t *he);
void comm_destroy(Comm *c);
int launch_allgather_f16(Comm *c, int slot, const void *src_slice, void *dst_full, int n_total, hipStream_t stream, hipError_t *he);
int comm_world_of(const Comm *c);
constexpr int kCommMaxRanks = 8, kCommFlagStride = 16;
struct PeerGatherEpi {
    unsigned char *peer[8];
    unsigned *epochs;
    void *dst;
    int rank, world, slot, slots;
    unsigned slice_elems;
    size_t vec_bytes, flags_off;
    unsigned long long timeout_ticks;
};
int comm_peer_gather_epi(Comm *c, int slot, void *dst_full, int n_total, PeerGatherEpi *out);
int comm_rccl_unique_id(void *id128);
int comm_rccl_init(Comm *c, const void *id128);
bool comm_has_rccl(const Comm *c);
const char *comm_rccl_last_error();
bool comm_peer_regime(const Comm *c, int n_total);
int launch_allgather_rccl(Comm *c, const void *src_slice, void *dst_full, size_t n_per_rank, hipStream_t stream);
size_t allgather_rows_workspace_bytes(int M, int n_total);
int launch_allgather_rows_f16(Comm *c, int slot, const void *src, void *dst, int M, int n_total, int ldd, void *workspace, hipStream_t stream, hipError_t *he);
void set_attention_fast_target(int wgs);
void set_attention_fast_waves(int nw);
void set_attention_fast_fuse(int r);
void set_attention_fast_probe_no_combine(int on);
void describe_attention_decode_fast(int heads, int keys, int *chunk, int *chunks, int *waves, int kv_heads = 0);
size_t attention_decode_workspace_bytes(int heads, int max_keys, int hd);
int launch_opt_attention_decode(const void *q, const void *kn, const void *vn, void *kc, void *vtc, const float *mask, void *out, int heads, int hd, int m, int pos,
                                int max_keys, int ld, float a_qk, float a_pv, hipStream_t stream, hipError_t *hip_err);
size_t attention_prefill_workspace_bytes(int heads, int m, int hd);
void set_attention_prefill_waves(int w);
int launch_attention_prefill(const void *qkv, int ld_qkv, void *kc, void *vc, const void *cosv, const void *sinv, const void *mask, int ld_mask, int causal,
                             void *out, int ld_out, void *workspace, int heads, int kv_heads, int max_keys, int pos, int m, float alpha, hipStream_t stream,
                             hipError_t *hip_err);
size_t attention_prefill_paged_workspace_bytes(int heads, int total_rows, int hd);
int describe_attention_prefill_paged(int heads, int causal, const int *segments, int nseg, int *form, int *pair, int *nblocks, int *workgroups);
int launch_attention_prefill_paged(const void *qkv, int ld_qkv, void *k_pool, void *v_pool, const int *table, int table_stride, int page_keys, const void *cosv,
                                   const void *sinv, int causal, void *out, int ld_out, void *workspace, int heads, int kv_heads, const int *segments, int nseg,
                                   int total_rows, float alpha, hipStream_t stream, hipError_t *hip_err);
struct AttnDeferred {
    int slots;
    int chunk;
    int heads;
    int stride;
    const float *part;
};
constexpr int kAttnDeferMaxSlots = 8;
int launch_attention_decode_fast(const void *qkv, void *kc, void *vc, const void *cosv, const void *sinv, const void *mask, void *out, void *workspace,
                                 int heads, int kv_heads, int hd, int max_keys, int pos, unsigned short alpha_bits, hipStream_t stream, hipError_t *hip_err,
                                 const int *pos_dev = nullptr, AttnDeferred *deferred = nullptr);
void describe_attention_decode_batch(int heads, int kv_heads, int pos_bound, int *chunk, int *chunks, int *waves);
size_t attention_decode_batch_workspace_bytes(int batch, int heads, int max_keys, int hd);
int launch_attention_decode_batch(const void *qkv, void *kc, void *vc, const void *cosv, const void *sinv, void *out, void *workspace, int batch, int heads,
                                  int kv_heads, int hd, int max_keys, const int *pos_dev, int pos_bound, unsigned short alpha_bits, hipStream_t stream,
                                  hipError_t *hip_err);
size_t kv_pages_pool_bytes(int num_pages, int kv_heads, int page_keys, int hd);
int launch_attention_decode_paged(const void *qkv, void *k_pool, void *v_pool, const int *table, int table_stride, int page_keys, const void *cosv, const void *sinv,
                                  void *out, void *workspace, int batch, int heads, int kv_heads, int hd, const int *pos_dev, int pos_bound, unsigned short alpha_bits,
                                  hipStream_t stream, hipError_t *hip_err);
int launch_kv_pages_copy(bool gather, void *k_lin, void *v_lin, void *k_pool, void *v_pool, const int *table_row, int page_keys, int num_pages, int kv_heads,
                         int lin_max_keys, int key0, int nkeys, hipStream_t stream, hipError_t *hip_err);
int launch_kv_block_table_check(const int *table, int table_stride, int page_keys, int num_pages, int batch, const int *pos_dev, int pos_bound, unsigned *violations,
                                hipStream_t stream, hipError_t *hip_err);
int launch_rope_half(void *q, void *k, const void *cosv, const void *sinv, int heads, int len, int hd, int start_idx, hipStream_t stream, hipError_t *hip_err);
int launch_softmax_half(const void *x, void *out, long long rows, int n, hipStream_t stream, hipError_t *hip_err);
int launch_prefetch(const void *ptr, long long bytes, int workgroups, hipStream_t stream, hipError_t *hip_err);
int launch_add_half(const void *a, const void *b, void *c, long long n, hipStream_t stream, hipError_t *hip_err);
int launch_silu_mul_half(void *a, const void *b, long long n, hipStream_t stream, hipError_t *hip_err);

}
```

Baseline: 1039 tokens/s.

## Restructure token kernel into producer wave with LDS ring feeding consumer waves

Replaces the 16-wave token kernel, where every wave loaded its own weight units into registers, with one producer wave that streams weight and scale chunks into an 11-slot LDS ring through buffer-to-LDS DMA, and seven consumer waves that convert activations and run the int8 MFMA reductions from the ring. Full and free flags in LDS, with bounded waits, coordinate the two sides. Stage records are now read through the constant address space instead of being copied into LDS. The goal is to keep more HBM traffic in flight per workgroup and separate loading from compute. The cost is fewer compute waves, spin-wait overhead and a much larger LDS footprint, which can lower occupancy. Lab-only timing rungs are also added.

Result: no change. 1039 tokens/s (median of 2 runs) (+0.0%).

```diff
diff --git a/tinychatengine_amd/csrc/tce_capi.hip b/tinychatengine_amd/csrc/tce_capi.hip
--- a/tinychatengine_amd/csrc/tce_capi.hip
+++ b/tinychatengine_amd/csrc/tce_capi.hip
@@ -183,6 +183,13 @@
     }
     if (mode >= 7710 && mode <= 7710 + 512) {
         tce::set_i8_token_max_units(mode - 7710);
+        return TCE_OK;
+    }
+    if (mode >= 7704 && mode <= 7706) {
+#ifndef TCE_LAB
+        if (mode != 7704) return fail(TCE_ERR_BAD_ARG, "debug modes 7705 / 7706 (the token engine's timing rungs) need the lab build (python -m tinychatengine_amd.build --lab, TCE_LIB_PATH)");
+#endif
+        tce::set_i8_token_rung(mode - 7704);
         return TCE_OK;
     }
     if (mode >= 7700 && mode <= 7703) {
@@ -1686,8 +1693,8 @@
 int tce_plan_geometry(const tce_plan *plan, int *rows, int *depth, int *waves, int *workgroups) {
     if (plan && plan->token_i8 && rows && depth && waves && workgroups) {
         *rows = plan->token_i8_taken;
-        *depth = 1;
-        *waves = 16;
+        *depth = tce::i8_token_plan_ring_slots();
+        *waves = tce::i8_token_plan_waves();
         *workgroups = tce::i8_token_plan_blocks(plan->token_i8);
         return TCE_OK;
     }
diff --git a/tinychatengine_amd/csrc/w4a16_gemv_i8_token.hip b/tinychatengine_amd/csrc/w4a16_gemv_i8_token.hip
--- a/tinychatengine_amd/csrc/w4a16_gemv_i8_token.hip
+++ b/tinychatengine_amd/csrc/w4a16_gemv_i8_token.hip
@@ -5,14 +5,30 @@
 #include <new>
 #include <vector>
 
+#ifndef TCE_TOK_CONSUMERS
+#define TCE_TOK_CONSUMERS 7
+#endif
+#ifndef TCE_TOK_AHEAD
+#define TCE_TOK_AHEAD 2
+#endif
+
 namespace tce {
 
 namespace {
 
-constexpr int kTokWaves = 16;
+constexpr int kTokConsumers = TCE_TOK_CONSUMERS;
+constexpr int kTokWaves = 1 + kTokConsumers;
 constexpr int kTokMaxChunks = 15;
 constexpr int kTokMaxUnits = 512;
 constexpr int kTokMaxTiles = 128;
+constexpr int kTokRing = 11;
+constexpr int kTokAhead = TCE_TOK_AHEAD;
+constexpr int kTokDmaPerFill = 9;
+constexpr int kTokConvPerWave = (kTokMaxChunks + kTokConsumers - 1) / kTokConsumers;
+constexpr int kTokRed = 64;
+static_assert(kTokRing >= kTokAhead + 1 + 3 && kTokAhead * kTokDmaPerFill < 64, "ring depth / the vmcnt field");
+static_assert(kTokRed >= kTokMaxChunks + kTokConsumers + kTokRing && (kTokRed & (kTokRed - 1)) == 0, "partial rows in progress");
+static_assert(kTokConsumers >= 1 && kTokConsumers <= 15, "waves per workgroup");
 
 struct TokSeg {
     const void *words;
@@ -28,23 +44,28 @@
     int K, U, nch, nseg, ntiles, pad;
     TokSeg seg[TCE_MAX_GROUP];
 };
-constexpr int kRecWords = sizeof(TokStage) / 4;
-static_assert(sizeof(TokStage) % 8 == 0 && kRecWords <= 128, "a record is fetched by one wave, 8 bytes per lane");
+typedef const __attribute__((address_space(4))) TokStage *tok_stage_ptr;
+typedef const __attribute__((address_space(4))) TokSeg *tok_seg_ptr;
 
 struct TokArgs {
     const TokStage *stages;
     int n_stages;
+    int rung;
     unsigned *status;
     const unsigned *epoch;
     unsigned long long *dbg;
 };
 
-constexpr int kPlanesBytes = kTokMaxChunks * 4096;
-constexpr int kRecOff = kPlanesBytes;
-constexpr int kShOff = kRecOff + 3 * (int)sizeof(TokStage);
-constexpr int kCntOff = kShOff + 128;
-constexpr int kRedOff = kCntOff + kTokMaxTiles * 4;
-constexpr int kLdsBytes = kRedOff + kTokMaxUnits * 64;
+constexpr int kSlotBytes = 8192 + 256;
+constexpr int kRingOff = 0;
+constexpr int kPlanesOff = kRingOff + kTokRing * kSlotBytes;
+constexpr int kRedOff = kPlanesOff + kTokMaxChunks * 4096;
+constexpr int kCtlOff = kRedOff + kTokRed * 64;
+constexpr int kwFull = 0, kwFree = 16, kwReady = 32, kwSh = 48, kwCnt = 80, kwDone = kwCnt + kTokRed, kCtlWords = kwDone + 16;
+constexpr int kLdsBytes = kCtlOff + kCtlWords * 4;
+static_assert(kPlanesOff % 16 == 0 && kRedOff % 16 == 0 && kLdsBytes <= 160 * 1024 && kTokRing <= 16, "LDS layout");
+
+typedef __attribute__((address_space(3))) void tok_lds_void_t;
 
 template <int DPP_CTRL, int ROW_MASK = 0xF>
 __device__ __forceinline__ unsigned tok_dpp_max_u32(unsigned v) {
@@ -68,320 +89,454 @@
     return reinterpret_cast<T *>(((unsigned long long)hi << 32) | lo);
 }
 
+__device__ __forceinline__ unsigned tok_peek(unsigned lds_byte_addr) {
+    unsigned v;
+    asm volatile("ds_read_b32 %0, %1\n\ts_waitcnt lgkmcnt(0)" : "=v"(v) : "v"(lds_byte_addr) : "memory");
+    return (unsigned)__builtin_amdgcn_readfirstlane((int)v);
+}
+__device__ __forceinline__ void tok_poke(unsigned lds_byte_addr, unsigned v) {
+    asm volatile("ds_write_b32 %0, %1\n\ts_waitcnt lgkmcnt(0)" ::"v"(lds_byte_addr), "v"(v) : "memory");
+}
+template <int N>
+__device__ __forceinline__ void tok_wait_vmcnt() {
+    asm volatile("s_waitcnt vmcnt(%0)" ::"n"(N) : "memory");
+}
+
+template <typename Pred, typename Idle>
+__device__ __forceinline__ void tok_bounded_wait(Pred ok, Idle idle, bool &dead, unsigned *status) {
+    if (dead || ok()) return;
+    unsigned tries = 0;
+    unsigned long long t0 = 0;
+    for (;;) {
+        idle();
+        if (ok()) return;
+        if ((++tries & 255u) == 0u) {
+            if (__hip_atomic_load(status, __ATOMIC_RELAXED, __HIP_MEMORY_SCOPE_AGENT) != 0u) {
+                dead = true;
+                return;
+            }
+            const unsigned long long now = wall_clock64();
+            if (t0 == 0) t0 = now;
+            else if (now - t0 > 30000000ull) {
+                __hip_atomic_store(status, 1u, __ATOMIC_RELAXED, __HIP_MEMORY_SCOPE_AGENT);
+                dead = true;
+                return;
+            }
+        }
+    }
+}
+
 template <bool STAMPS>
 __global__ __launch_bounds__(64 * kTokWaves) void w4a16_gemv_i8_token_kernel(const TokArgs args) {
     extern __shared__ __attribute__((aligned(16))) unsigned char smem[];
     const int tid = threadIdx.x;
     const int lane = tid & 63;
     const int w = __builtin_amdgcn_readfirstlane(tid >> 6);
-    const int kq = lane >> 4, j16 = lane & 15;
-    const int p_l = j16 & 3, uu_l = j16 >> 2;
     const int P = gridDim.x, b = blockIdx.x;
     const int n = args.n_stages;
-    unsigned *const planes_all = reinterpret_cast<unsigned *>(smem);
-    TokStage *const rec = reinterpret_cast<TokStage *>(smem + kRecOff);
-    int *const shx = reinterpret_cast<int *>(smem + kShOff);
-    unsigned *const tile_cnt = reinterpret_cast<unsigned *>(smem + kCntOff);
-    float *const red = reinterpret_cast<float *>(smem + kRedOff);
-    const unsigned tag = (unsigned)__builtin_amdgcn_readfirstlane((int)__hip_atomic_load(args.epoch, __ATOMIC_RELAXED, __HIP_MEMORY_SCOPE_AGENT)) << 16;
+#ifdef TCE_LAB
+    const int rung = args.rung;
+#else
+    constexpr int rung = 0;
+#endif
+    const tok_stage_ptr stages = (tok_stage_ptr)(unsigned long long)args.stages;
+    const unsigned lds0 = (unsigned)(unsigned long long)(tok_lds_void_t *)smem;
+    const unsigned ctl = lds0 + kCtlOff;
     unsigned long long *const stamps = STAMPS && args.dbg ? args.dbg + (size_t)b * n * 8 : nullptr;
     auto stamp = [&](int s, int i) {
         if constexpr (STAMPS) {
-            if (stamps && tid == 0) stamps[s * 8 + i] = wall_clock64();
+            if (stamps && lane == 0) stamps[s * 8 + i] = wall_clock64();
         }
     };
-
-    if (tid < kRecWords) reinterpret_cast<unsigned *>(&rec[0])[tid] = reinterpret_cast<const unsigned *>(args.stages)[tid];
+    bool dead = false;
+
+    if (tid < kCtlWords) reinterpret_cast<unsigned *>(smem + kCtlOff)[tid] = 0u;
     __syncthreads();
 
-    uint4_t wq[8];
-    uint2_t sc[2];
+    if (w == 0) {
+        int slot = 0, pub_slot = 0, pending = 0;
+        unsigned turn = 1, pub_turn = 1;
+        auto publish = [&]() {
+            tok_poke(ctl + (kwFull + pub_slot) * 4, pub_turn);
+            if (++pub_slot == kTokRing) pub_slot = 0, ++pub_turn;
+            --pending;
+        };
+        auto wait_oldest = [&]() {
+            static_assert(kTokAhead <= 6, "one case per depth");
+            switch (pending) {
+                case 1: tok_wait_vmcnt<0>(); break;
+                case 2: tok_wait_vmcnt<1 * kTokDmaPerFill>(); break;
+                case 3: tok_wait_vmcnt<2 * kTokDmaPerFill>(); break;
+                case 4: tok_wait_vmcnt<3 * kTokDmaPerFill>(); break;
+                case 5: tok_wait_vmcnt<4 * kTokDmaPerFill>(); break;
+                default: tok_wait_vmcnt<5 * kTokDmaPerFill>(); break;
+            }
+        };
+        for (int s = 0; s < n; ++s) {
+            const tok_stage_ptr R = stages + s;
+            const int U = R->U, nch = R->nch, nseg = R->nseg, ntiles = R->ntiles;
+            const int ntw = b < ntiles ? (ntiles - 1 - b) / P + 1 : 0;
+            for (int i = 0; i < ntw; ++i) {
+                const int t = b + i * P;
+                int si = 0;
+                for (int q = 1; q < nseg; ++q)
+                    if (t >= R->seg[q].tile_begin) si = q;
+                const tok_seg_ptr S = &R->seg[si];
+                const int tl = t - S->tile_begin;
+                const __amdgpu_buffer_rsrc_t rs_w = __builtin_amdgcn_make_buffer_rsrc(const_cast<void *>(S->words), 0, S->bytes_w, 0x00020000);
+                const __amdgpu_buffer_rsrc_t rs_none = __builtin_amdgcn_make_buffer_rsrc(const_cast<void *>(S->words), 0, 0, 0x00020000);
+                const __amdgpu_buffer_rsrc_t rs_s = __builtin_amdgcn_make_buffer_rsrc(const_cast<half_t *>(S->dscales), 0, S->bytes_s, 0x00020000);
+                for (int c = 0; c < nch; ++c) {
+                    const unsigned want = turn - 1u;
+                    const unsigned a_free = ctl + (kwFree + slot) * 4;
+                    tok_bounded_wait([&]() { return tok_peek(a_free) == want; },
+                                     [&]() {
+                                         if (pending > 0) {
+                                             wait_oldest();
+                                             publish();
+                                         } else {
+                                             __builtin_amdgcn_s_sleep(1);
+                                         }
+                                     },
+                                     dead, args.status);
+                    const int u0 = c * 8;
+                    unsigned char *dst = smem + kRingOff + slot * kSlotBytes;
+#pragma unroll
+                    for (int tt = 0; tt < 8; ++tt)
+                        __builtin_amdgcn_raw_ptr_buffer_load_lds(u0 + tt < U ? rs_w : rs_none, (tok_lds_void_t *)(dst + tt * 1024), 16, lane * 16, (tl * U + u0 + tt) * 1024, 0,  2);
+                    __builtin_amdgcn_raw_ptr_buffer_load_lds(rs_s, (tok_lds_void_t *)(dst + 8192), 4, lane * 4, (tl * U + u0) * 32, 0, 0);
+                    if constexpr (STAMPS) {
+                        if (i == 0 && c == 0) stamp(s, 0);
+                        if (i == ntw - 1 && c == nch - 1) stamp(s, 1);
+                    }
+                    if (++slot == kTokRing) slot = 0, ++turn;
+                    if (++pending > kTokAhead) {
+                        tok_wait_vmcnt<kTokAhead * kTokDmaPerFill>();
+                        publish();
+                    }
+                }
+            }
+        }
+        tok_wait_vmcnt<0>();
+        while (pending > 0) publish();
+        return;
+    }
+
+    const int ci = w - 1;
+    const int kq = lane >> 4, j16 = lane & 15;
+    const int p_l = j16 & 3, uu_l = j16 >> 2;
+    unsigned *const planes_all = reinterpret_cast<unsigned *>(smem + kPlanesOff);
+    int *const shx = reinterpret_cast<int *>(smem + kCtlOff + kwSh * 4);
+    unsigned *const tile_cnt = reinterpret_cast<unsigned *>(smem + kCtlOff + kwCnt * 4);
+    unsigned *const done_cnt = reinterpret_cast<unsigned *>(smem + kCtlOff + kwDone * 4);
+    float *const red = reinterpret_cast<float *>(smem + kRedOff);
+    const unsigned tag = (unsigned)__builtin_amdgcn_readfirstlane((int)__hip_atomic_load(args.epoch, __ATOMIC_RELAXED, __HIP_MEMORY_SCOPE_AGENT)) << 16;
     const int4_t zero4 = int4_t{0, 0, 0, 0};
-
+    auto nap = []() { __builtin_amdgcn_s_sleep(1); };
+
+    int gbase = 0, tbase = 0;
+    int g_next = ci;
+    int slot = ci % kTokRing;
+    unsigned turn = 1u + (unsigned)(ci / kTokRing);
     for (int s = 0; s < n; ++s) {
-        const TokStage *R = &rec[s % 3];
-        const int K = sgpr(R->K), U = sgpr(R->U), nch = sgpr(R->nch), nseg = sgpr(R->nseg), ntiles = sgpr(R->ntiles);
+        const tok_stage_ptr R = stages + s;
+        const int K = R->K, U = R->U, nch = R->nch, nseg = R->nseg, ntiles = R->ntiles;
         const int ntw = b < ntiles ? (ntiles - 1 - b) / P + 1 : 0;
         const int nunits = ntw * nch;
-        stamp(s, 0);
-
-        const int rec_pair = (lane * 2 < kRecWords ? lane * 2 : kRecWords - 2);
-        const uint2_t recv = *reinterpret_cast<const uint2_t *>(reinterpret_cast<const unsigned *>(args.stages + (s + 1 < n ? s + 1 : n - 1)) + rec_pair);
-
         auto seg_of = [&](int t) {
             int si = 0;
             for (int q = 1; q < nseg; ++q)
-                if (t >= sgpr(R->seg[q].tile_begin)) si = q;
+                if (t >= R->seg[q].tile_begin) si = q;
             return si;
         };
-        auto request = [&](int u) {
-            const int i = u / nch, c = u - i * nch;
-            const int t = b + i * P;
-            const TokSeg *S = &R->seg[seg_of(t)];
-            const int tl = t - sgpr(S->tile_begin);
-            const int u0 = c * 8;
-            const __amdgpu_buffer_rsrc_t rs_w = __builtin_amdgcn_make_buffer_rsrc(const_cast<void *>(sgpr_ptr(S->words)), 0, sgpr(S->bytes_w), 0x00020000);
-            const __amdgpu_buffer_rsrc_t rs_none = __builtin_amdgcn_make_buffer_rsrc(const_cast<void *>(sgpr_ptr(S->words)), 0, 0, 0x00020000);
-            const __amdgpu_buffer_rsrc_t rs_s = __builtin_amdgcn_make_buffer_rsrc(const_cast<half_t *>(sgpr_ptr(S->dscales)), 0, sgpr(S->bytes_s), 0x00020000);
-#pragma unroll
-            for (int ps = 0; ps < 2; ++ps) {
-                const int ga = tl * U + u0 + ps * 4 + uu_l;
-                sc[ps] = __builtin_bit_cast(uint2_t, __builtin_amdgcn_raw_buffer_load_b64(rs_s, (ga * 16 + 4 * kq) * 2, 0, 0));
-            }
-#pragma unroll
-            for (int tt = 0; tt < 8; ++tt)
-                wq[tt] = __builtin_amdgcn_raw_buffer_load_b128(u0 + tt < U ? rs_w : rs_none, lane * 16, (tl * U + u0 + tt) * 1024,  2);
-        };
-        int u_cur = w;
-        const int u_first = u_cur;
-        if (u_cur < nunits) request(u_cur);
-        __builtin_amdgcn_sched_barrier(0);
-
-        uint4_t xv[2];
-        xv[0] = xv[1] = uint4_t{0u, 0u, 0u, 0u};
-        if (w < nch) {
-            const unsigned *A_tag = sgpr_ptr(R->A_tag);
+
+        if (rung != 1 && nunits > 0 && ci < nch) {
+            tok_bounded_wait([&]() { return tok_peek(ctl + kwDone * 4) >= (unsigned)gbase; }, nap, dead, args.status);
+            uint4_t xa[kTokConvPerWave][2];
+            const unsigned *A_tag = rung == 2 ? nullptr : R->A_tag;
             if (A_tag == nullptr) {
-                const __amdgpu_buffer_rsrc_t rs_x = __builtin_amdgcn_make_buffer_rsrc(const_cast<half_t *>(sgpr_ptr(R->A)), 0, K * 2, 0x00020000);
-#pragma unroll
-                for (int c = 0; c < 2; ++c) xv[c] = __builtin_amdgcn_raw_buffer_load_b128(rs_x, w * 2048 + (lane + 64 * c) * 16, 0, 0);
+                const __amdgpu_buffer_rsrc_t rs_x = __builtin_amdgcn_make_buffer_rsrc(const_cast<half_t *>(R->A), 0, K * 2, 0x00020000);
+#pragma unroll
+                for (int j = 0; j < kTokConvPerWave; ++j)
+#pragma unroll
+                    for (int h = 0; h < 2; ++h) xa[j][h] = __builtin_amdgcn_raw_buffer_load_b128(rs_x, (ci + j * kTokConsumers) * 2048 + (lane + 64 * h) * 16, 0, 0);
             } else {
                 const __amdgpu_buffer_rsrc_t rs_t = __builtin_amdgcn_make_buffer_rsrc(const_cast<unsigned *>(A_tag), 0, K * 4, 0x00020000);
-                bool need[2];
-                uint4_t lo[2], hi[2];
-#pragma unroll
-                for (int c = 0; c < 2; ++c) {
-                    need[c] = w * 1024 + (lane + 64 * c) * 8 < K;
-                    lo[c] = hi[c] = uint4_t{tag, tag, tag, tag};
-                }
+                bool need[kTokConvPerWave][2];
+                uint4_t lo[kTokConvPerWave][2], hi[kTokConvPerWave][2];
+#pragma unroll
+                for (int j = 0; j < kTokConvPerWave; ++j)
+#pragma unroll
+                    for (int h = 0; h < 2; ++h) {
+                        need[j][h] = (ci + j * kTokConsumers) * 1024 + (lane + 64 * h) * 8 < K;
+                        lo[j][h] = hi[j][h] = uint4_t{tag, tag, tag, tag};
+                    }
                 int tries = 0;
                 for (;;) {
 #pragma unroll
-                    for (int c = 0; c < 2; ++c)
-                        if (need[c]) {
-                            lo[c] = __builtin_amdgcn_raw_buffer_load_b128(rs_t, w * 4096 + (lane + 64 * c) * 32, 0,  17);
-                            hi[c] = __builtin_amdgcn_raw_buffer_load_b128(rs_t, w * 4096 + (lane + 64 * c) * 32 + 16, 0,  17);
-                        }
+                    for (int j = 0; j < kTokConvPerWave; ++j)
+#pragma unroll
+                        for (int h = 0; h < 2; ++h)
+                            if (need[j][h]) {
+                                lo[j][h] = __builtin_amdgcn_raw_buffer_load_b128(rs_t, (ci + j * kTokConsumers) * 4096 + (lane + 64 * h) * 32, 0,  17);
+                                hi[j][h] = __builtin_amdgcn_raw_buffer_load_b128(rs_t, (ci + j * kTokConsumers) * 4096 + (lane + 64 * h) * 32 + 16, 0,  17);
+                            }
                     bool again = false;
 #pragma unroll
-                    for (int c = 0; c < 2; ++c)
-                        if (need[c]) {
-                            const unsigned bad = ((lo[c].x ^ tag) | (lo[c].y ^ tag) | (lo[c].z ^ tag) | (lo[c].w ^ tag) | (hi[c].x ^ tag) | (hi[c].y ^ tag) | (hi[c].z ^ tag) |
-                                                  (hi[c].w ^ tag)) >> 16;
-                            need[c] = bad != 0u;
-                            again |= need[c];
-                        }
-                    if (!__builtin_amdgcn_ballot_w64(again)) break;
+                    for (int j = 0; j < kTokConvPerWave; ++j)
+#pragma unroll
+                        for (int h = 0; h < 2; ++h)
+                            if (need[j][h]) {
+                                const unsigned bad = ((lo[j][h].x ^ tag) | (lo[j][h].y ^ tag) | (lo[j][h].z ^ tag) | (lo[j][h].w ^ tag) | (hi[j][h].x ^ tag) | (hi[j][h].y ^ tag) |
+                                                      (hi[j][h].z ^ tag) | (hi[j][h].w ^ tag)) >> 16;
+                                need[j][h] = bad != 0u;
+                                again |= need[j][h];
+                            }
+                    if (!__builtin_amdgcn_ballot_w64(again) || dead) break;
                     __builtin_amdgcn_s_sleep(2);
                     if ((++tries & 255) == 0) {
-                        if (__hip_atomic_load(args.status, __ATOMIC_RELAXED, __HIP_MEMORY_SCOPE_AGENT) != 0u) break;
+                        if (__hip_atomic_load(args.status, __ATOMIC_RELAXED, __HIP_MEMORY_SCOPE_AGENT) != 0u) {
+                            dead = true;
+                            break;
+                        }
                         if (tries > (1 << 18)) {
                             __hip_atomic_store(args.status, 1u, __ATOMIC_RELAXED, __HIP_MEMORY_SCOPE_AGENT);
+                            dead = true;
                             break;
                         }
                     }
                 }
 #pragma unroll
-                for (int c = 0; c < 2; ++c)
-                    xv[c] = uint4_t{(lo[c].x & 0xFFFFu) | (lo[c].y << 16), (lo[c].z & 0xFFFFu) | (lo[c].w << 16), (hi[c].x & 0xFFFFu) | (hi[c].y << 16),
-                                    (hi[c].z & 0xFFFFu) | (hi[c].w << 16)};
-            }
-            asm volatile("" : "+v"(xv[0]), "+v"(xv[1]));
+                for (int j = 0; j < kTokConvPerWave; ++j)
+#pragma unroll
+                    for (int h = 0; h < 2; ++h)
+                        xa[j][h] = uint4_t{(lo[j][h].x & 0xFFFFu) | (lo[j][h].y << 16), (lo[j][h].z & 0xFFFFu) | (lo[j][h].w << 16), (hi[j][h].x & 0xFFFFu) | (hi[j][h].y << 16),
+                                           (hi[j][h].z & 0xFFFFu) | (hi[j][h].w << 16)};
+            }
+            if constexpr (STAMPS) {
+                asm volatile("" : "+v"(xa[0][0]), "+v"(xa[0][1]));
+                if (ci == 0) stamp(s, 5);
+            }
+#pragma unroll
+            for (int j = 0; j < kTokConvPerWave; ++j) {
+                const int c = ci + j * kTokConsumers;
+                if (c >= nch) break;
+                uint4_t xv[2] = {xa[j][0], xa[j][1]};
+                unsigned mx = 0;
+#pragma unroll
+                for (int h = 0; h < 2; ++h)
+#pragma unroll
+                    for (int q = 0; q < 4; ++q) {
+                        const unsigned v = xv[h][q] & 0x7FFF7FFFu;
+                        const unsigned v2 = v << 16;
+                        const unsigned m2 = v > v2 ? v : v2;
+                        mx = mx > m2 ? mx : m2;
+                    }
+                mx = tok_dpp_max_u32<0x111>(mx);
+                mx = tok_dpp_max_u32<0x112>(mx);
+                mx = tok_dpp_max_u32<0x114>(mx);
+                mx = tok_dpp_max_u32<0x118>(mx);
+                mx = tok_dpp_max_u32<0x142, 0xA>(mx);
+                mx = tok_dpp_max_u32<0x143, 0xC>(mx);
+                const int E = (int)((unsigned)__builtin_amdgcn_readlane((int)mx, 63) >> 26);
+                const int sh = 44 - E;
+                if (lane == 0) {
+                    shx[c] = sh;
+                    shx[16 + c] = E == 31 ? 1 : 0;
+                }
+                const float scale = __builtin_bit_cast(float, (unsigned)(127 + sh) << 23);
+                unsigned *planes = planes_all + c * 1024;
+#pragma unroll
+                for (int h2 = 0; h2 < 2; ++h2) {
+                    unsigned d[8];
+#pragma unroll
+                    for (int q = 0; q < 4; ++q) {
+                        const half_t lo = __builtin_bit_cast(half_t, (unsigned short)(xv[h2][q] & 0xFFFFu));
+                        const half_t hi = __builtin_bit_cast(half_t, (unsigned short)(xv[h2][q] >> 16));
+                        d[2 * q] = ((unsigned)(int)__builtin_fmaf((float)lo, scale, 0.0f) + 0x00808080u) ^ 0x00808080u;
+                        d[2 * q + 1] = ((unsigned)(int)__builtin_fmaf((float)hi, scale, 0.0f) + 0x00808080u) ^ 0x00808080u;
+                    }
+                    const int cc = lane + 64 * h2;
+                    const int tu = cc >> 4, sw = (cc >> 2) & 3, q4 = cc & 3;
+#pragma unroll
+                    for (int h = 0; h < 2; ++h) {
+                        const unsigned a0 = d[2 * h], a1 = d[2 * h + 4], a2 = d[2 * h + 1], a3 = d[2 * h + 5];
+                        const unsigned t0 = __builtin_amdgcn_perm(a1, a0, 0x05010400u);
+                        const unsigned t1 = __builtin_amdgcn_perm(a1, a0, 0x07030602u);
+                        const unsigned t2 = __builtin_amdgcn_perm(a3, a2, 0x05010400u);
+                        const unsigned t3 = __builtin_amdgcn_perm(a3, a2, 0x07030602u);
+                        const int base = (((tu * 2 + h) * 4) * 4 + q4) * 4 + sw;
+                        planes[base + 0] = __builtin_amdgcn_perm(t2, t0, 0x05040100u);
+                        planes[base + 16] = __builtin_amdgcn_perm(t2, t0, 0x07060302u);
+                        planes[base + 32] = __builtin_amdgcn_perm(t3, t1, 0x05040100u);
+                        planes[base + 48] = __builtin_amdgcn_perm(t3, t1, 0x07060302u);
+                    }
+                }
+                tok_poke(ctl + (kwReady + c) * 4, (unsigned)(s + 1));
+                if constexpr (STAMPS) {
+                    if (c == 0) stamp(s, 3);
+                    if (c == nch - 1) stamp(s, 6);
+                }
+            }
         }
-        stamp(s, 1);
-        lds_barrier();
-        stamp(s, 2);
-        if (tid < kTokMaxTiles) tile_cnt[tid] = 0u;
-        if (w < nch) {
-            unsigned mx = 0;
-#pragma unroll
-            for (int c = 0; c < 2; ++c)
+
+        while (g_next < gbase + nunits) {
+            const int u = g_next - gbase;
+            const int i = u / nch, c = u - i * nch;
+            const int u0 = c * 8;
+            const unsigned a_full = ctl + (kwFull + slot) * 4;
+            const unsigned my_turn = turn;
+            tok_bounded_wait([&]() { return tok_peek(a_full) == my_turn; }, nap, dead, args.status);
+            if constexpr (STAMPS) {
+                if (u == 0) stamp(s, 2);
+            }
+            uint4_t wq[8];
+            uint2_t sc[2];
+            if (rung != 1) {
+                const unsigned char *src = smem + kRingOff + slot * kSlotBytes;
+#pragma unroll
+                for (int tt = 0; tt < 8; ++tt) wq[tt] = *reinterpret_cast<const uint4_t *>(src + tt * 1024 + lane * 16);
+#pragma unroll
+                for (int ps = 0; ps < 2; ++ps) {
+                    sc[ps] = *reinterpret_cast<const uint2_t *>(src + 8192 + ((ps * 4 + uu_l) * 16 + 4 * kq) * 2);
+                    if (u0 + ps * 4 + uu_l >= U) sc[ps] = uint2_t{0u, 0u};
+                }
+                asm volatile("s_waitcnt lgkmcnt(0)" : "+v"(wq[0]), "+v"(wq[1]), "+v"(wq[2]), "+v"(wq[3]), "+v"(wq[4]), "+v"(wq[5]), "+v"(wq[6]), "+v"(wq[7]), "+v"(sc[0]), "+v"(sc[1])::"memory");
+            }
+            tok_poke(ctl + (kwFree + slot) * 4, my_turn);
+            slot += kTokConsumers;
+            while (slot >= kTokRing) slot -= kTokRing, ++turn;
+            if (rung != 1) {
+                const unsigned a_ready = ctl + (kwReady + c) * 4;
+                tok_bounded_wait([&]() { return tok_peek(a_ready) == (unsigned)(s + 1); }, nap, dead, args.status);
+                const int t = b + i * P;
+                const tok_seg_ptr S = &R->seg[seg_of(t)];
+                const int tl = t - S->tile_begin;
+                const int N = S->N, epi = S->epilogue;
+                half_t *C = S->C;
+                const int row = tl * 16 + (lane & 15);
+                unsigned short oldc = 0;
+                if ((epi & TCE_W4_ADD_TO_C) && lane < 16 && row < N) oldc = __hip_atomic_load(reinterpret_cast<unsigned short *>(C) + row, __ATOMIC_RELAXED, __HIP_MEMORY_SCOPE_AGENT);
+                const unsigned *planes = planes_all + c * 1024;
+                int4_t B[4][2];
+#pragma unroll
+                for (int uu = 0; uu < 4; ++uu) B[uu][0] = B[uu][1] = zero4;
+                auto read_b = [&](int ps) {
+#pragma unroll
+                    for (int uu = 0; uu < 4; ++uu)
+                        if (uu_l == uu) {
+#pragma unroll
+                            for (int h = 0; h < 2; ++h) {
+                                const unsigned *src = planes + (((((ps * 4 + uu) * 2 + h) * 4 + p_l) * 4 + kq) * 4);
+                                B[uu][h] = __builtin_bit_cast(int4_t, *reinterpret_cast<const uint4_t *>(src));
+                            }
+                        }
+                };
+                read_b(0);
+                float acc[4] = {0.f, 0.f, 0.f, 0.f};
+#pragma unroll
+                for (int ps = 0; ps < 2; ++ps) {
+                    int4_t dd0 = zero4, dd1 = zero4;
+#pragma unroll
+                    for (int uu = 0; uu < 4; ++uu) {
+                        const int t = ps * 4 + uu;
+                        int4_t alo, ahi;
+#pragma unroll
+                        for (int q = 0; q < 4; ++q) {
+                            const unsigned x = wq[t][q];
+                            ahi[q] = (int)((x & 0xF0F0F0F0u) ^ 0x80808080u);
+                            alo[q] = (int)(((x << 4) & 0xF0F0F0F0u) ^ 0x80808080u);
+                        }
+                        dd0 = __builtin_amdgcn_mfma_i32_16x16x64_i8(alo, B[uu][0], dd0, 0, 0, 0);
+                        dd1 = __builtin_amdgcn_mfma_i32_16x16x64_i8(ahi, B[uu][1], dd1, 0, 0, 0);
+                    }
+                    const half_t s0 = __builtin_bit_cast(half_t, (unsigned short)(sc[ps][0] & 0xFFFFu));
+                    const half_t s1 = __builtin_bit_cast(half_t, (unsigned short)(sc[ps][0] >> 16));
+                    const half_t s2 = __builtin_bit_cast(half_t, (unsigned short)(sc[ps][1] & 0xFFFFu));
+                    const half_t s3 = __builtin_bit_cast(half_t, (unsigned short)(sc[ps][1] >> 16));
+                    const int4_t tot = dd0 + dd1;
+                    acc[0] = __builtin_fmaf((float)tot[0], (float)s0, acc[0]);
+                    acc[1] = __builtin_fmaf((float)tot[1], (float)s1, acc[1]);
+                    acc[2] = __builtin_fmaf((float)tot[2], (float)s2, acc[2]);
+                    acc[3] = __builtin_fmaf((float)tot[3], (float)s3, acc[3]);
+                    if (ps == 0) read_b(1);
+                }
+                const int sh_c = sgpr(shx[c]);
+                const bool bad_c = sgpr(shx[16 + c]) != 0;
+                const float cj = bad_c ? __builtin_nanf("") : __builtin_bit_cast(float, (unsigned)(127 + 8 * p_l - sh_c - 4) << 23);
+                float *pslot = red + (size_t)(g_next & (kTokRed - 1)) * 16;
 #pragma unroll
                 for (int q = 0; q < 4; ++q) {
-                    const unsigned v = xv[c][q] & 0x7FFF7FFFu;
-                    const unsigned v2 = v << 16;
-                    const unsigned m2 = v > v2 ? v : v2;
-                    mx = mx > m2 ? mx : m2;
-                }
-            mx = tok_dpp_max_u32<0x111>(mx);
-            mx = tok_dpp_max_u32<0x112>(mx);
-            mx = tok_dpp_max_u32<0x114>(mx);
-            mx = tok_dpp_max_u32<0x118>(mx);
-            mx = tok_dpp_max_u32<0x142, 0xA>(mx);
-            mx = tok_dpp_max_u32<0x143, 0xC>(mx);
-            const int E = (int)((unsigned)__builtin_amdgcn_readlane((int)mx, 63) >> 26);
-            const int sh = 44 - E;
-            if (lane == 0) {
-                shx[w] = sh;
-                shx[16 + w] = E == 31 ? 1 : 0;
-            }
-            const float scale = __builtin_bit_cast(float, (unsigned)(127 + sh) << 23);
-            unsigned *planes = planes_all + w * 1024;
-#pragma unroll
-            for (int c = 0; c < 2; ++c) {
-                unsigned d[8];
-#pragma unroll
-                for (int q = 0; q < 4; ++q) {
-                    const half_t lo = __builtin_bit_cast(half_t, (unsigned short)(xv[c][q] & 0xFFFFu));
-                    const half_t hi = __builtin_bit_cast(half_t, (unsigned short)(xv[c][q] >> 16));
-                    d[2 * q] = ((unsigned)(int)__builtin_fmaf((float)lo, scale, 0.0f) + 0x00808080u) ^ 0x00808080u;
-                    d[2 * q + 1] = ((unsigned)(int)__builtin_fmaf((float)hi, scale, 0.0f) + 0x00808080u) ^ 0x00808080u;
-                }
-                const int cc = lane + 64 * c;
-                const int tu = cc >> 4, sw = (cc >> 2) & 3, q4 = cc & 3;
-#pragma unroll
-                for (int h = 0; h < 2; ++h) {
-                    const unsigned a0 = d[2 * h], a1 = d[2 * h + 4], a2 = d[2 * h + 1], a3 = d[2 * h + 5];
-                    const unsigned t0 = __builtin_amdgcn_perm(a1, a0, 0x05010400u);
-                    const unsigned t1 = __builtin_amdgcn_perm(a1, a0, 0x07030602u);
-                    const unsigned t2 = __builtin_amdgcn_perm(a3, a2, 0x05010400u);
-                    const unsigned t3 = __builtin_amdgcn_perm(a3, a2, 0x07030602u);
-                    const int base = (((tu * 2 + h) * 4) * 4 + q4) * 4 + sw;
-                    planes[base + 0] = __builtin_amdgcn_perm(t2, t0, 0x05040100u);
-                    planes[base + 16] = __builtin_amdgcn_perm(t2, t0, 0x07060302u);
-                    planes[base + 32] = __builtin_amdgcn_perm(t3, t1, 0x05040100u);
-                    planes[base + 48] = __builtin_amdgcn_perm(t3, t1, 0x07060302u);
-                }
-            }
+                    float v = acc[q] * cj;
+                    v = tok_dpp_add_f32<0xB1>(v);
+                    v = tok_dpp_add_f32<0x4E>(v);
+                    v = tok_dpp_add_f32<0x128>(v);
+                    v = tok_dpp_add_f32<0x124>(v);
+                    if (j16 == 0) pslot[kq * 4 + q] = v;
+                }
+                asm volatile("s_waitcnt lgkmcnt(0)" ::: "memory");
+                unsigned *cnt = tile_cnt + ((tbase + i) & (kTokRed - 1));
+                unsigned old = 0;
+                if (lane == 0) old = __hip_atomic_fetch_add(cnt, 1u, __ATOMIC_RELAXED, __HIP_MEMORY_SCOPE_WORKGROUP);
+                asm volatile("" ::: "memory");
+                const bool last = (unsigned)__builtin_amdgcn_readfirstlane((int)old) == (unsigned)(nch - 1);
+                if (last) {
+                    if (lane == 0) *cnt = 0u;
+                    stamp(s, 4);
+                    unsigned *C_tag = S->C_tag;
+                    const int g0 = gbase + i * nch;
+                    float part[kTokMaxChunks];
+#pragma unroll
+                    for (int k2 = 0; k2 < kTokMaxChunks; ++k2) {
+                        const int kk = k2 < nch ? k2 : nch - 1;
+                        part[k2] = red[(size_t)((g0 + kk) & (kTokRed - 1)) * 16 + (lane & 15)];
+                    }
+                    float v = 0.f;
+#pragma unroll
+                    for (int k2 = 0; k2 < kTokMaxChunks; ++k2) v += k2 < nch ? part[k2] : 0.f;
+                    half_t y = (half_t)v;
+                    const half_t y_other = __builtin_bit_cast(half_t, (unsigned short)tok_dpp_u32<0xB1>((unsigned)__builtin_bit_cast(unsigned short, y)));
+                    int idx = row;
+                    bool live = lane < 16 && row < N;
+                    if (epi & TCE_W4_SILU_MUL_PAIRS) {
+                        y = silu_mul_half(y, y_other);
+                        idx = row >> 1;
+                        live = live && (lane & 1) == 0;
+                    } else if (epi & TCE_W4_ADD_TO_C) {
+                        y = __builtin_bit_cast(half_t, oldc) + y;
+                    }
+                    const unsigned short bits = __builtin_bit_cast(unsigned short, y);
+                    if (live) {
+                        if (epi & TCE_W4_ADD_TO_C) __hip_atomic_store(reinterpret_cast<unsigned short *>(C) + idx, bits, __ATOMIC_RELAXED, __HIP_MEMORY_SCOPE_AGENT);
+                        else C[idx] = y;
+                    }
+                    if (C_tag) {
+                        const unsigned word = tag | bits;
+                        const __amdgpu_buffer_rsrc_t rs_c = __builtin_amdgcn_make_buffer_rsrc(C_tag, 0, 0x7FFFFFF0, 0x00020000);
+                        if (epi & TCE_W4_SILU_MUL_PAIRS) {
+                            const unsigned w1 = tok_dpp_u32<0x102>(word), w2 = tok_dpp_u32<0x104>(word), w3 = tok_dpp_u32<0x106>(word);
+                            if (lane < 16 && (lane & 7) == 0 && row + 7 < N) {
+                                __builtin_amdgcn_raw_buffer_store_b128(uint4_t{word, w1, w2, w3}, rs_c, idx * 4, 0,  17);
+                            } else if (lane < 16 && row < N && (lane & 1) == 0 && !(((row & ~7) + 7) < N)) {
+                                __hip_atomic_store(C_tag + idx, word, __ATOMIC_RELAXED, __HIP_MEMORY_SCOPE_AGENT);
+                            }
+                        } else {
+                            const unsigned w1 = tok_dpp_u32<0x101>(word), w2 = tok_dpp_u32<0x102>(word), w3 = tok_dpp_u32<0x103>(word);
+                            if (lane < 16 && (lane & 3) == 0 && row + 3 < N) {
+                                __builtin_amdgcn_raw_buffer_store_b128(uint4_t{word, w1, w2, w3}, rs_c, idx * 4, 0,  17);
+                            } else if (lane < 16 && row < N && !(((row & ~3) + 3) < N)) {
+                                __hip_atomic_store(C_tag + idx, word, __ATOMIC_RELAXED, __HIP_MEMORY_SCOPE_AGENT);
+                            }
+                        }
+                    }
+                }
+            }
+            asm volatile("s_waitcnt lgkmcnt(0)" ::: "memory");
+            if (lane == 0) (void)__hip_atomic_fetch_add(done_cnt, 1u, __ATOMIC_RELAXED, __HIP_MEMORY_SCOPE_WORKGROUP);
+            g_next += kTokConsumers;
         }
-        lds_barrier();
-        stamp(s, 3);
-        *reinterpret_cast<uint2_t *>(reinterpret_cast<unsigned *>(&rec[(s + 1) % 3]) + rec_pair) = recv;
-
-        while (u_cur < nunits) {
-            const int i = u_cur / nch, c = u_cur - i * nch;
-            const unsigned *planes = planes_all + c * 1024;
-            int4_t B[4][2];
-#pragma unroll
-            for (int uu = 0; uu < 4; ++uu) B[uu][0] = B[uu][1] = zero4;
-            auto read_b = [&](int ps) {
-#pragma unroll
-                for (int uu = 0; uu < 4; ++uu)
-                    if (uu_l == uu) {
-#pragma unroll
-                        for (int h = 0; h < 2; ++h) {
-                            const unsigned *src = planes + (((((ps * 4 + uu) * 2 + h) * 4 + p_l) * 4 + kq) * 4);
-                            B[uu][h] = __builtin_bit_cast(int4_t, *reinterpret_cast<const uint4_t *>(src));
-                        }
-                    }
-            };
-            read_b(0);
-            if constexpr (STAMPS) {
-                if (u_cur == u_first) {
-                    asm volatile("s_waitcnt vmcnt(0)" ::: "memory");
-                    stamp(s, 5);
-                }
-            }
-            float acc[4] = {0.f, 0.f, 0.f, 0.f};
-#pragma unroll
-            for (int ps = 0; ps < 2; ++ps) {
-                int4_t dd0 = zero4, dd1 = zero4;
-#pragma unroll
-                for (int uu = 0; uu < 4; ++uu) {
-                    const int t = ps * 4 + uu;
-                    int4_t alo, ahi;
-#pragma unroll
-                    for (int q = 0; q < 4; ++q) {
-                        const unsigned x = wq[t][q];
-                        ahi[q] = (int)((x & 0xF0F0F0F0u) ^ 0x80808080u);
-                        alo[q] = (int)(((x << 4) & 0xF0F0F0F0u) ^ 0x80808080u);
-                    }
-                    dd0 = __builtin_amdgcn_mfma_i32_16x16x64_i8(alo, B[uu][0], dd0, 0, 0, 0);
-                    dd1 = __builtin_amdgcn_mfma_i32_16x16x64_i8(ahi, B[uu][1], dd1, 0, 0, 0);
-                }
-                const half_t s0 = __builtin_bit_cast(half_t, (unsigned short)(sc[ps][0] & 0xFFFFu));
-                const half_t s1 = __builtin_bit_cast(half_t, (unsigned short)(sc[ps][0] >> 16));
-                const half_t s2 = __builtin_bit_cast(half_t, (unsigned short)(sc[ps][1] & 0xFFFFu));
-                const half_t s3 = __builtin_bit_cast(half_t, (unsigned short)(sc[ps][1] >> 16));
-                const int4_t tot = dd0 + dd1;
-                acc[0] = __builtin_fmaf((float)tot[0], (float)s0, acc[0]);
-                acc[1] = __builtin_fmaf((float)tot[1], (float)s1, acc[1]);
-                acc[2] = __builtin_fmaf((float)tot[2], (float)s2, acc[2]);
-                acc[3] = __builtin_fmaf((float)tot[3], (float)s3, acc[3]);
-                if (ps == 0) read_b(1);
-            }
-            const int sh_c = sgpr(shx[c]);
-            const bool bad_c = sgpr(shx[16 + c]) != 0;
-            const float cj = bad_c ? __builtin_nanf("") : __builtin_bit_cast(float, (unsigned)(127 + 8 * p_l - sh_c - 4) << 23);
-            float *slot = red + (size_t)u_cur * 16;
-            if constexpr (STAMPS) {
-                if (u_cur == u_first) {
-                    asm volatile("" : "+v"(acc[0]), "+v"(acc[1]), "+v"(acc[2]), "+v"(acc[3]));
-                    stamp(s, 6);
-                }
-            }
-#pragma unroll
-            for (int q = 0; q < 4; ++q) {
-                float v = acc[q] * cj;
-                v = tok_dpp_add_f32<0xB1>(v);
-                v = tok_dpp_add_f32<0x4E>(v);
-                v = tok_dpp_add_f32<0x128>(v);
-                v = tok_dpp_add_f32<0x124>(v);
-                if (j16 == 0) slot[kq * 4 + q] = v;
-            }
-            asm volatile("s_waitcnt lgkmcnt(0)" ::: "memory");
-            unsigned old = 0;
-            if (lane == 0) old = __hip_atomic_fetch_add(tile_cnt + i, 1u, __ATOMIC_RELAXED, __HIP_MEMORY_SCOPE_WORKGROUP);
-            asm volatile("" ::: "memory");
-            const bool last = (unsigned)__builtin_amdgcn_readfirstlane((int)old) == (unsigned)(nch - 1);
-            if constexpr (STAMPS) {
-                if (u_cur == u_first) stamp(s, 7);
-            }
-            const int t = b + i * P;
-            if (last) {
-                if constexpr (STAMPS) {
-                    if (stamps && lane == 0) stamps[s * 8 + 4] = wall_clock64();
-                }
-                const TokSeg *S = &R->seg[seg_of(t)];
-                const int tl = t - sgpr(S->tile_begin);
-                const int N = sgpr(S->N), epi = sgpr(S->epilogue);
-                half_t *C = sgpr_ptr(S->C);
-                unsigned *C_tag = sgpr_ptr(S->C_tag);
-                const float *parts = red + (size_t)(i * nch) * 16 + (lane & 15);
-                float v = 0.f;
-                for (int k2 = 0; k2 < nch; ++k2) v += parts[k2 * 16];
-                const int row = tl * 16 + (lane & 15);
-                half_t y = (half_t)v;
-                const half_t y_other = __builtin_bit_cast(half_t, (unsigned short)tok_dpp_u32<0xB1>((unsigned)__builtin_bit_cast(unsigned short, y)));
-                int idx = row;
-                bool live = lane < 16 && row < N;
-                if (epi & TCE_W4_SILU_MUL_PAIRS) {
-                    y = silu_mul_half(y, y_other);
-                    idx = row >> 1;
-                    live = live && (lane & 1) == 0;
-                } else if (epi & TCE_W4_ADD_TO_C) {
-                    unsigned short oldc = 0;
-                    if (live) oldc = __hip_atomic_load(reinterpret_cast<unsigned short *>(C) + row, __ATOMIC_RELAXED, __HIP_MEMORY_SCOPE_AGENT);
-                    y = __builtin_bit_cast(half_t, oldc) + y;
-                }
-                const unsigned short bits = __builtin_bit_cast(unsigned short, y);
-                if (live) {
-                    if (epi & TCE_W4_ADD_TO_C) __hip_atomic_store(reinterpret_cast<unsigned short *>(C) + idx, bits, __ATOMIC_RELAXED, __HIP_MEMORY_SCOPE_AGENT);
-                    else C[idx] = y;
-                }
-                if (C_tag) {
-                    const unsigned word = tag | bits;
-                    const __amdgpu_buffer_rsrc_t rs_c = __builtin_amdgcn_make_buffer_rsrc(C_tag, 0, 0x7FFFFFF0, 0x00020000);
-                    if (epi & TCE_W4_SILU_MUL_PAIRS) {
-                        const unsigned w1 = tok_dpp_u32<0x102>(word), w2 = tok_dpp_u32<0x104>(word), w3 = tok_dpp_u32<0x106>(word);
-                        if (lane < 16 && (lane & 7) == 0 && row + 7 < N) {
-                            __builtin_amdgcn_raw_buffer_store_b128(uint4_t{word, w1, w2, w3}, rs_c, idx * 4, 0,  17);
-                        } else if (lane < 16 && row < N && (lane & 1) == 0 && !(((row & ~7) + 7) < N)) {
-                            __hip_atomic_store(C_tag + idx, word, __ATOMIC_RELAXED, __HIP_MEMORY_SCOPE_AGENT);
-                        }
-                    } else {
-                        const unsigned w1 = tok_dpp_u32<0x101>(word), w2 = tok_dpp_u32<0x102>(word), w3 = tok_dpp_u32<0x103>(word);
-                        if (lane < 16 && (lane & 3) == 0 && row + 3 < N) {
-                            __builtin_amdgcn_raw_buffer_store_b128(uint4_t{word, w1, w2, w3}, rs_c, idx * 4, 0,  17);
-                        } else if (lane < 16 && row < N && !(((row & ~3) + 3) < N)) {
-                            __hip_atomic_store(C_tag + idx, word, __ATOMIC_RELAXED, __HIP_MEMORY_SCOPE_AGENT);
-                        }
-                    }
-                }
-            }
-            u_cur += kTokWaves;
-            if (u_cur < nunits) request(u_cur);
-        }
+        gbase += nunits;
+        tbase += ntw;
     }
 }
 
@@ -397,6 +552,7 @@
 thread_local unsigned long long *g_tok_stamps = nullptr;
 thread_local int g_tok_mode = 0;
 thread_local int g_tok_max_units = kTokMaxUnits;
+thread_local int g_tok_rung = 0;
 
 }
 
@@ -404,7 +560,7 @@
     TokStage *stages = nullptr;
     unsigned *sync = nullptr;
     unsigned *shadow = nullptr;
-    int n = 0, blocks = 0;
+    int n = 0, blocks = 0, rung = 0;
     unsigned long long *stamps = nullptr;
 };
 
@@ -422,6 +578,9 @@
 
 int i8_token_plan_stages(const I8TokenPlan *tp) { return tp ? tp->n : 0; }
 int i8_token_plan_blocks(const I8TokenPlan *tp) { return tp ? tp->blocks : 0; }
+int i8_token_plan_ring_slots() { return kTokRing; }
+int i8_token_plan_waves() { return kTokWaves; }
+void set_i8_token_rung(int rung) { g_tok_rung = rung == 1 || rung == 2 ? rung : 0; }
 
 int i8_token_plan_create(const tce_w4a16_desc *descs, const int32_t *groups, int n_launches, I8TokenPlan **out, int *n_taken, hipError_t *hip_err) {
     if (g_tok_mode == 1) return TCE_ERR_UNSUPPORTED_SHAPE;
@@ -494,6 +653,7 @@
     tp->blocks = P;
 #ifdef TCE_LAB
     tp->stamps = g_tok_stamps;
+    tp->rung = g_tok_rung;
 #endif
     auto n_out_of = [&](const TokStage &L, int i) { return (L.seg[i].epilogue & TCE_W4_SILU_MUL_PAIRS) ? L.seg[i].N / 2 : L.seg[i].N; };
     size_t words = 0;
@@ -588,6 +748,7 @@
     a.n_stages = tp->n;
     a.status = tp->sync;
     a.epoch = tp->sync + 1;
+    a.rung = tp->rung;
     a.dbg = tp->stamps;
     const dim3 grid(tp->blocks), block(64 * kTokWaves);
 #ifdef TCE_LAB
diff --git a/tinychatengine_amd/csrc/w4a16_kernels.hpp b/tinychatengine_amd/csrc/w4a16_kernels.hpp
--- a/tinychatengine_amd/csrc/w4a16_kernels.hpp
+++ b/tinychatengine_amd/csrc/w4a16_kernels.hpp
@@ -115,6 +115,9 @@
 int i8_token_plan_status(I8TokenPlan *tp, unsigned *status, hipError_t *hip_err);
 int i8_token_plan_stages(const I8TokenPlan *tp);
 int i8_token_plan_blocks(const I8TokenPlan *tp);
+int i8_token_plan_ring_slots();
+int i8_token_plan_waves();
+void set_i8_token_rung(int rung);
 void i8_token_plan_destroy(I8TokenPlan *tp);
 void set_i8_token_stamps(void *buf);
 void set_i8_token_max_units(int u);
```
